# serval/kaboodle

Hardware: AMD Instinct MI355X
Metric: simulated peer-rounds/sec (whole node) + rounds to fingerprint convergence (higher is better)
Workload: dtype u8

## Files before the change

include/kaboodle_sim.h:

```cpp
#ifndef KABOODLE_SIM_H
#define KABOODLE_SIM_H

#include <stddef.h>
#include <stdint.h>

#ifdef __cplusplus
extern "C" {
#endif

#define KB_ABI_VERSION 3u

enum {
  KB_OK = 0,
  KB_INVALID_OPERATION = 1,
  KB_IO_ERROR = 2,
  KB_NO_DEVICE = 3,
  KB_STOPPING_FAILED = 4,
  KB_INVALID_ARGUMENT = 5,
  KB_CAPACITY = 6
};

enum { KB_INIT_JOIN = 0,
       KB_INIT_CONVERGED = 1 };

enum { KB_FAILED_SIM_SENDER = 0,
       KB_FAILED_SOCKET_FAITHFUL = 1 };

typedef struct kb_config {
  uint32_t abi_version;
  uint32_t capacity;
  uint32_t initial_nodes;
  uint32_t init_mode;
  uint64_t seed;
  uint32_t loss_threshold;
  uint32_t churn_threshold;
  int32_t  fault_end_round;
  uint32_t max_waves;
  uint32_t failed_mode;
  uint32_t id_len;
  uint32_t partition_groups;
  int32_t  partition_start;
  int32_t  partition_end;
  int32_t  device;
  uint32_t debug_flags;
  uint32_t track_latency;
  uint32_t variant;
  uint32_t sparse_row_cap;
  uint32_t stat_flags;
  uint32_t reserved[1];
} kb_config;
enum { KB_STAT_NO_SF_FAILED_DROPS = 1u };
enum { KB_VARIANT_SAME_WINDOW_BCAST = 1u,
       KB_VARIANT_EXACT_LRU = 2u,
       KB_VARIANT_SPARSE_ROWS = 4u };

enum {
  KB_DBG_PHASEB_HBM = 1u,
  KB_DBG_RESP_HBM = 2u,
  KB_DBG_KP_HBM = 4u,
  KB_DBG_KP_BIG_SMALL = 8u,
  KB_DBG_PROC_UNSORTED = 16u,
  KB_DBG_WAVE_GRAPH = 32u,
  KB_DBG_RESP_WAVE_HBM = 64u,
  KB_DBG_NO_UNION = 128u,
  KB_DBG_A3X_KPL8 = 256u,
  KB_DBG_A3X_WIDE = 512u,
  KB_DBG_WAVE0_SERIAL = 1024u
};

enum { KB_STATE_KNOWN = 0, KB_STATE_WAITING_FOR_PING = 1, KB_STATE_WAITING_FOR_INDIRECT_PING = 2 };
typedef struct kb_peer_state {
  uint32_t peer;
  uint32_t state;
  int32_t  since;
  uint32_t latency_ms;
  uint32_t identity_len;
  uint8_t  identity[32];
} kb_peer_state;
#define KB_LATENCY_NONE 0xFFFFFFFFu

typedef struct kb_stats {
  int32_t  round;
  uint32_t alive;
  uint32_t agree;
  int32_t  first_converged_round;
  int32_t  last_converged_round;
  uint32_t next_free_id;
  uint64_t sent_ping, sent_ping_req, sent_ack, sent_known_peers, sent_kpr;
  uint64_t bcast_join, bcast_failed;
  uint64_t drop_dead, drop_loss, drop_window, drop_oversize, drop_partition, drop_bcast;
  uint64_t removed_timeout, removed_failed, join_responses, curious_overflow, churn_leaves, churn_joins;
  uint64_t sent_kp_ids;
  uint64_t alive_rounds;
  uint64_t probe_responses;
  uint64_t exported;
  uint64_t reserved[4];
} kb_stats;

typedef struct kb_sim kb_sim;

void kb_config_default(kb_config* cfg);

int  kb_sim_create(const kb_config* cfg, kb_sim** out);
int  kb_sim_destroy(kb_sim* sim);
int  kb_sim_step(kb_sim* sim, uint32_t rounds);

int  kb_sim_start_node(kb_sim* sim, uint32_t node);
int  kb_sim_stop_node(kb_sim* sim, uint32_t node);
int  kb_sim_restart_node(kb_sim* sim, uint32_t node, uint32_t* new_node);
int  kb_sim_is_running(kb_sim* sim, uint32_t node, int* running);
int  kb_sim_ping_addrs(kb_sim* sim, uint32_t node, const uint32_t* peers, size_t n);
int  kb_sim_set_identity(kb_sim* sim, uint32_t node, const uint8_t* identity, size_t len);
int  kb_sim_identity(kb_sim* sim, uint32_t node, uint8_t* buf, size_t cap, size_t* len);

int  kb_sim_fingerprint(kb_sim* sim, uint32_t node, uint32_t* fp);
int  kb_sim_fingerprints(kb_sim* sim, uint32_t* fps, size_t cap);
int  kb_sim_peers(kb_sim* sim, uint32_t node, uint32_t* peers, size_t cap, size_t* n);
int  kb_sim_peer_states(kb_sim* sim, uint32_t node, kb_peer_state* out, size_t cap, size_t* n);
int  kb_sim_stats(kb_sim* sim, kb_stats* out);
int  kb_sim_true_fingerprint(kb_sim* sim, uint32_t* fp);

int  kb_sim_watch(kb_sim* sim, uint32_t node);
int  kb_sim_events(kb_sim* sim, uint32_t node, uint32_t* discovered, size_t cap_d, size_t* n_d,
                   uint32_t* departed, size_t cap_p, size_t* n_p, uint32_t* fp, int* fp_changed);

typedef struct kb_wire_addr { uint8_t ip[4]; uint16_t port; uint16_t pad; } kb_wire_addr;

typedef struct kb_probe_response {
  uint32_t responder;
  uint32_t probe;
  int32_t  round;
  kb_wire_addr prober;
  uint32_t identity_len;
  uint8_t  identity[32];
} kb_probe_response;
int  kb_sim_probe(kb_sim* sim, const kb_wire_addr* prober);
int  kb_sim_probe_responses(kb_sim* sim, kb_probe_response* out, size_t cap, size_t* n);
typedef struct kb_broadcast { uint32_t kind, sender, peer, pad; } kb_broadcast;
int  kb_sim_broadcasts(kb_sim* sim, kb_broadcast* out, size_t cap, size_t* n);

typedef struct kb_unicast {
  int32_t  round;
  uint32_t wave, sender, dest, seq, kind, a, fp, n, pay_off, pay_len, pad;
} kb_unicast;
int  kb_sim_set_external(kb_sim* sim, uint32_t node);
int  kb_sim_inject(kb_sim* sim, const kb_unicast* msg, const uint32_t* ids);
int  kb_sim_exported(kb_sim* sim, kb_unicast* out, size_t cap, size_t* n, uint32_t* ids, size_t cap_ids, size_t* n_ids);

#define KB_UNIQUE_ID_BYTES 128
int  kb_rccl_unique_id(uint8_t* out, size_t cap);
int  kb_ipc_unique_id(uint8_t* out, size_t cap);
int  kb_sim_create_rank(const kb_config* cfg, int32_t rank, int32_t world, const uint8_t* unique_id,
                        kb_sim** out);
int  kb_sim_create_local(const kb_config* cfg, int32_t shards, kb_sim** out);
int  kb_sim_shard_info(kb_sim* sim, int32_t* rank, int32_t* world, uint32_t* lo, uint32_t* hi);

int  kb_sim_dump_row(kb_sim* sim, uint32_t node, uint8_t* row, size_t cap);
int  kb_sim_dump_scalars(kb_sim* sim, int32_t* out, size_t cap);
int  kb_sim_dump_suspects(kb_sim* sim, uint32_t node, int32_t* out, size_t cap, size_t* n);
int  kb_sim_debug_paths(kb_sim* sim, uint32_t* mask);
int  kb_sim_debug_counters(kb_sim* sim, uint64_t* out, size_t cap);
int  kb_sim_dump_curious(kb_sim* sim, uint32_t node, int32_t* out, size_t cap, size_t* n);
int  kb_sim_sparse_footprint(kb_sim* sim, uint64_t* out, size_t cap);
int  kb_sim_dump_checkpoints(kb_sim* sim, uint32_t node, uint32_t seg[128], uint64_t* stale, uint32_t* dirty,
                             uint32_t* fp_cached);
enum { KB_FOLD_TICK = 0, KB_FOLD_FP_ALL = 1, KB_FOLD_FP_ONE = 2, KB_FOLD_THREAD = 3 };
typedef struct kb_fold_probe {
  uint32_t path, split, nrows, pad;
  const uint32_t* rows;
  const uint8_t*  running;
  const uint32_t* bits;
  const uint64_t* stale;
  const uint32_t* segp_in;
  uint32_t* segp_out;
  uint64_t* stale_out;
  uint32_t* dirty_out;
  uint32_t* fp_out;
  uint64_t* fold_bytes;
} kb_fold_probe;
int  kb_sim_debug_fold(kb_sim* sim, const kb_fold_probe* p);

int  kb_format_addr(uint32_t id, char* buf, size_t cap);
uint32_t kb_fingerprint_of_set(const uint32_t* ids, size_t n, const uint8_t* identities,
                               size_t id_stride, const uint8_t* id_lens);

const char* kb_last_error(void);

enum { KB_WIRE_PING = 0, KB_WIRE_PING_REQUEST = 1, KB_WIRE_ACK = 2, KB_WIRE_KNOWN_PEERS = 3,
       KB_WIRE_KNOWN_PEERS_REQUEST = 4,
       KB_WIRE_JOIN = 16, KB_WIRE_FAILED = 17, KB_WIRE_PROBE = 18,
       KB_WIRE_PROBE_RESPONSE = 32 };
enum { KB_WIRE_CHANNEL_UNICAST = 0, KB_WIRE_CHANNEL_BROADCAST = 1, KB_WIRE_CHANNEL_PROBE_RESPONSE = 2 };
typedef struct kb_wire_entry { kb_wire_addr addr; uint32_t id_off, id_len; } kb_wire_entry;
typedef struct kb_wire_msg {
  uint32_t kind;
  uint32_t identity_off, identity_len;
  kb_wire_addr peer;
  uint32_t fingerprint, num_peers;
  uint32_t n_entries;
} kb_wire_msg;
int kb_wire_encode(const kb_wire_msg* m, const kb_wire_entry* entries, const uint8_t* idents, uint8_t* buf,
                   size_t cap, size_t* size);
int kb_wire_decode(const uint8_t* buf, size_t len, int channel, kb_wire_msg* m, kb_wire_entry* entries, size_t cap);
int kb_wire_addr_of_id(uint32_t id, kb_wire_addr* out);
int kb_wire_id_of_addr(const kb_wire_addr* addr, uint32_t* id);

enum { KB_KT_ROWPASS = 0,
       KB_KT_ROUND = 1,
       KB_KT_FOLD = 2,
       KB_KT_RESP = 3,
       KB_KT_PROC = 4 };
int  kb_sim_kernel_time(kb_sim* sim, int kind, double* ms, uint64_t* launches);
int  kb_sim_reset_kernel_time(kb_sim* sim);
int  kb_sim_kernel_bytes(kb_sim* sim, int kind, uint64_t* bytes);
#define KB_WAVE_SLOTS 9
typedef struct kb_kernel_time {
  char     name[24];
  double   ms;
  uint64_t launches;
  uint64_t bytes;
// ... 12 lines not shown
```

kaboodle_amd/_ffi.py:

```python
from __future__ import annotations

import ctypes as C
import os
from dataclasses import dataclass

KB_ABI_VERSION = 3
KB_OK, KB_INVALID_OPERATION, KB_IO_ERROR, KB_NO_DEVICE, KB_STOPPING_FAILED, KB_INVALID_ARGUMENT, KB_CAPACITY = range(7)
KB_INIT_JOIN, KB_INIT_CONVERGED = 0, 1
KB_FAILED_SIM_SENDER, KB_FAILED_SOCKET_FAITHFUL = 0, 1
KB_DBG_PHASEB_HBM, KB_DBG_RESP_HBM, KB_DBG_KP_HBM, KB_DBG_KP_BIG_SMALL, KB_DBG_PROC_UNSORTED = 1, 2, 4, 8, 16
KB_DBG_ALL = 31
KB_DBG_WAVE_GRAPH = 32
KB_DBG_RESP_WAVE_HBM = 64
KB_DBG_NO_UNION = 128
KB_DBG_A3X_KPL8 = 256
KB_DBG_A3X_WIDE = 512
KB_DBG_WAVE0_SERIAL = 1024
KB_VARIANT_SAME_WINDOW_BCAST, KB_VARIANT_EXACT_LRU = 1, 2
KB_STAT_NO_SF_FAILED_DROPS = 1
KB_VARIANT_SPARSE_ROWS = 4
KB_LATENCY_NONE = 0xFFFFFFFF
KT_ROWPASS, KT_ROUND, KT_FOLD, KT_RESP, KT_PROC = 0, 1, 2, 3, 4
KB_WAVE_SLOTS = 9
STATE_NAMES = {0: "Known", 1: "WaitingForPing", 2: "WaitingForIndirectPing"}


class KbConfig(C.Structure):
    _fields_ = [
        ("abi_version", C.c_uint32), ("capacity", C.c_uint32), ("initial_nodes", C.c_uint32),
        ("init_mode", C.c_uint32), ("seed", C.c_uint64), ("loss_threshold", C.c_uint32),
        ("churn_threshold", C.c_uint32), ("fault_end_round", C.c_int32), ("max_waves", C.c_uint32),
        ("failed_mode", C.c_uint32), ("id_len", C.c_uint32), ("partition_groups", C.c_uint32),
        ("partition_start", C.c_int32), ("partition_end", C.c_int32), ("device", C.c_int32),
        ("debug_flags", C.c_uint32), ("track_latency", C.c_uint32), ("variant", C.c_uint32),
        ("sparse_row_cap", C.c_uint32), ("stat_flags", C.c_uint32), ("reserved", C.c_uint32 * 1),
    ]


class KbPeerState(C.Structure):
    _fields_ = [("peer", C.c_uint32), ("state", C.c_uint32), ("since", C.c_int32), ("latency_ms", C.c_uint32),
                ("identity_len", C.c_uint32), ("identity", C.c_uint8 * 32)]


PEER_STATE_DTYPE = [("peer", "<u4"), ("state", "<u4"), ("since", "<i4"), ("latency_ms", "<u4"), ("identity_len", "<u4"),
                    ("identity", "u1", (32,))]


class KbStats(C.Structure):
    _fields_ = [
        ("round", C.c_int32), ("alive", C.c_uint32), ("agree", C.c_uint32),
        ("first_converged_round", C.c_int32), ("last_converged_round", C.c_int32), ("next_free_id", C.c_uint32),
        ("sent_ping", C.c_uint64), ("sent_ping_req", C.c_uint64), ("sent_ack", C.c_uint64),
        ("sent_known_peers", C.c_uint64), ("sent_kpr", C.c_uint64),
        ("bcast_join", C.c_uint64), ("bcast_failed", C.c_uint64),
        ("drop_dead", C.c_uint64), ("drop_loss", C.c_uint64), ("drop_window", C.c_uint64),
        ("drop_oversize", C.c_uint64), ("drop_partition", C.c_uint64), ("drop_bcast", C.c_uint64),
        ("removed_timeout", C.c_uint64), ("removed_failed", C.c_uint64), ("join_responses", C.c_uint64),
        ("curious_overflow", C.c_uint64), ("churn_leaves", C.c_uint64), ("churn_joins", C.c_uint64),
        ("sent_kp_ids", C.c_uint64), ("alive_rounds", C.c_uint64), ("probe_responses", C.c_uint64),
        ("exported", C.c_uint64), ("reserved", C.c_uint64 * 4),
    ]

    def as_dict(self) -> dict:
        return {n: getattr(self, n) for n, _ in self._fields_ if n != "reserved"}


class KbKernelTime(C.Structure):
    _fields_ = [("name", C.c_char * 24), ("ms", C.c_double), ("launches", C.c_uint64), ("bytes", C.c_uint64),
                ("has_bytes", C.c_uint32), ("pad", C.c_uint32), ("wave_ms", C.c_double * KB_WAVE_SLOTS)]


KB_CENSUS_NONE = 0xFFFFFFFF


def _summary(st: C.Structure, lists=()) -> dict:
    return {n: [int(x) for x in getattr(st, n)] if n in lists else int(getattr(st, n))
            for n, _ in st._fields_ if n not in ("reserved", "pad")}


def diff_results(a, b, array_names) -> list[str]:
    import numpy as np
    out = [f"summary.{k}: {v} != {b.summary[k]}" for k, v in a.summary.items() if b.summary[k] != v]
    for name in array_names:
        x, y = getattr(a, name), getattr(b, name)
        if (x is None) != (y is None):
            out.append(f"{name}: only one side has the array")
        elif x is not None and not np.array_equal(x, y):
            if x.ndim > 1 or x.shape != y.shape:
                out.append(f"{name}: {len(x)} listed != {len(y)} listed, or other entries")
            else:
                bad = np.flatnonzero(x != y)
                out.append(f"{name}: {len(bad)} differ, first id {bad[0]}: {x[bad[0]]} != {y[bad[0]]}")
    return out


_PTR = {"u4": C.POINTER(C.c_uint32), "i4": C.POINTER(C.c_int32), "u8": C.POINTER(C.c_uint64)}


def _out_arrays(arrays: bool, *groups):
    import numpy as np
    outs, args = [], []
    for dtypes, n in groups:
        made = [np.zeros(n, dtype=dt) if arrays else None for dt in dtypes]
        outs += made
        args += [m.ctypes.data_as(_PTR[dt]) if arrays else None for m, dt in zip(made, dtypes)]
        args.append(n if arrays else 0)
    return outs, args


class KbCensus(C.Structure):
    _fields_ = [("round", C.c_int32), ("observers", C.c_uint32), ("running", C.c_uint32), ("exact_views", C.c_uint32),
                ("pairs", C.c_uint64), ("missing", C.c_uint64), ("stale", C.c_uint64),
                ("full_ids", C.c_uint32), ("ghost_ids", C.c_uint32), ("least_known", C.c_uint32),
                ("least_known_by", C.c_uint32), ("top_ghost", C.c_uint32), ("top_ghost_by", C.c_uint32),
                ("reserved", C.c_uint64 * 4)]

    def as_dict(self) -> dict:
        return _summary(self)


class KbReciprocity(C.Structure):
    _fields_ = [("round", C.c_int32), ("observers", C.c_uint32), ("mutual_pairs", C.c_uint64),
                ("oneway_pairs", C.c_uint64), ("rows_mutual", C.c_uint32), ("rows_oneway", C.c_uint32),
                ("max_mutual_row", C.c_uint32), ("max_mutual", C.c_uint32), ("pairs_listed", C.c_uint64),
                ("reserved", C.c_uint64 * 4)]

    def as_dict(self) -> dict:
        return _summary(self)


class KbFpClass(C.Structure):
    _fields_ = [("fp", C.c_uint32), ("size", C.c_uint32), ("rep", C.c_uint32), ("pad", C.c_uint32)]


class KbFpClasses(C.Structure):
    _fields_ = [("round", C.c_int32), ("observers", C.c_uint32), ("classes", C.c_uint32), ("largest", C.c_uint32),
                ("singletons", C.c_uint32), ("true_fp", C.c_uint32), ("true_size", C.c_uint32),
                ("true_rank", C.c_uint32), ("size_hist", C.c_uint32 * 32), ("listed", C.c_uint32),
                ("listed_observers", C.c_uint32), ("reserved", C.c_uint64 * 4)]

    def as_dict(self) -> dict:
        d = _summary(self, ("size_hist",))
        d["size_hist"] = d.pop("size_hist")
        return d


KB_FPC_LIST_MAX = 1024
_FPC_OUT = [C.POINTER(KbFpClasses), C.POINTER(KbFpClass), C.c_size_t, C.POINTER(C.c_size_t), C.POINTER(C.c_uint32),
            C.POINTER(C.c_uint32), C.c_size_t]


class KbLatCensus(C.Structure):
    _fields_ = [("round", C.c_int32), ("observers", C.c_uint32), ("measured", C.c_uint64), ("sum_ms", C.c_uint64),
                ("min_ms", C.c_uint32), ("max_ms", C.c_uint32), ("max_peer", C.c_uint32), ("measured_ids", C.c_uint32),
                ("hist", C.c_uint64 * 17), ("orphans", C.c_uint64), ("reserved", C.c_uint64 * 4)]

    def as_dict(self) -> dict:
        return _summary(self, ("hist",))


_LATC_OUT = [C.POINTER(KbLatCensus), C.POINTER(C.c_uint32), C.POINTER(C.c_uint64), C.POINTER(C.c_uint32),
             C.POINTER(C.c_uint32), C.c_size_t, C.POINTER(C.c_uint32), C.POINTER(C.c_uint64), C.c_size_t]


class KbAgeCensus(C.Structure):
    _fields_ = [("round", C.c_int32), ("observers", C.c_uint32), ("cells", C.c_uint64), ("suspects", C.c_uint64),
                ("ancient", C.c_uint64), ("windowed", C.c_uint64), ("fresh", C.c_uint64), ("dead_suspects", C.c_uint64),
                ("dead_ancient", C.c_uint64), ("dead_windowed", C.c_uint64), ("dead_fresh", C.c_uint64),
                ("unheard_ids", C.c_uint32), ("oldest_heard_id", C.c_uint32), ("oldest_heard", C.c_int32),
                ("pad", C.c_uint32), ("hist", C.c_uint64 * 256), ("reserved", C.c_uint64 * 4)]
# ... 773 lines not shown
```

kaboodle_amd/csrc/kb_common.h:

```cpp
#pragma once
#include "kb_device.h"
#include "../../include/kaboodle_sim.h"

namespace kb {

enum StatIdx {
  S_PING, S_PINGREQ, S_ACK, S_KP, S_KPR, S_BJOIN, S_BFAIL, S_DEAD, S_LOSS, S_WINDOW, S_OVERSIZE, S_PART, S_BDROP,
  S_RMTIMEOUT, S_RMFAILED, S_JRESP, S_CUROVF, S_CLEAVE, S_CJOIN,
  S_KPIDS,
  S_ROWB,
  S_FOLDB,
  S_A3ROWS, S_A3DEEP, S_A3CHUNKS,
  S_ALIVER,
  S_RESPB,
  S_PROCB,
  S_PROBERESP,
  S_EXPORT,
  S_A3X32, S_A3XCLAMP, S_A3XFEW, S_A3XLIVE, S_A3XWIDE,
  NSTAT
};
enum CtrIdx {
  C_KP, C_SLOW, C_ACTIVE, C_AGREE, C_ALIVE, C_LEAVES, C_NEXTFREE, C_ERR, C_FIRSTCONV, C_LASTCONV, C_LASTAGREE,
  C_LASTALIVE, C_DBG_INS, C_DBG_FP, C_DBG_MAXFP,
  C_DBG_KPR, C_DBG_KPRLOG, C_DBG_BASE,
  C_DBG_TNODE, C_DBG_TMAX, C_DBG_TBASE, C_DBG_TINS,
  C_DBG_TSTART, C_DBG_TEND, C_DBG_MSGS,
  C_TICK,
  C_ROUND,
  C_PATHS,
  C_DBG_SLOW_LONG, C_DBG_SLOW_NONMEM, C_DBG_SLOW_DIRTY, C_DBG_SLOW_KPR, C_DBG_SLOW_OTHER,
  C_RESTN,
  C_XREC, C_XPAY,
  NCTR
};
enum : uint32_t { PATH_PHASEB_HBM = 1, PATH_RESP_SCRATCH_SAMPLED = 2, PATH_RESP_SCRATCH_FULL = 4, PATH_KP_BIG_HBM = 8,
                  PATH_PROC_UNSORTED = 16, PATH_BFAIL_PREP_HBM = 32, PATH_RESP_WAVE = 64, PATH_KP_BIG_LDS = 128,
                  PATH_RESP_WAVE_HBM = 256,
                  PATH_PROC_DEFERRED = 512,
                  PATH_ROWPASS_LDS_HBM_LISTS = 1024,
                  PATH_KPR_WRAPPED = 2048,
                  PATH_RESP_JOINERS_HBM = 4096,
                  PATH_JOIN_LIST_PAST_UCAP = 8192 };
constexpr int NSEG = 64;
constexpr int ZT = 9;
constexpr int ZB = 9 * 1024;

struct Dev {
  uint32_t lo, hi;
  uint32_t C, W, SEGW, NWR;
  uint32_t segq, segm;
  uint32_t k0, k1;
  uint32_t loss_thr, churn_thr;
  int32_t fault_end;
  uint32_t failed_mode;
  uint32_t pgroups;
  int32_t pstart, pend;
  uint32_t uniform, L;
  uint32_t capk, capj;
  uint32_t paybound;
  uint32_t dbg;
  uint32_t dev;
  uint8_t* stamp;
  uint32_t* bits;
  uint2* segp;
  unsigned long long* sdirty;
  uint8_t* dirty;
  uint8_t* alive;
  uint8_t* idset;
  uint32_t* abits;
  int32_t* start_round;
  uint32_t* n;
  uint32_t* fp;
  int32_t* last_bcast;
  uint32_t* a3cur;
  Susp* susp;
  Cur* cur;
  uint32_t* paq;
  uint32_t* paq_n;
  uint32_t* cseg;
  uint32_t* segmul;
  uint32_t* seglen;
  uint32_t* zpow;
  uint32_t* zfin;
  uint32_t* ztab;
  uint32_t* zbtab;
  uint32_t* htab;
  unsigned long long* stats;
  unsigned long long* sacc;
  uint32_t* ctr;
  uint32_t* truefp;
  uint2* tfpart;
  uint32_t* flog;
  uint32_t* flog_n;
  uint32_t* fstart;
  int32_t* kpr_big;
  uint16_t* lat;
  int32_t wave;
  uint8_t* ext;
  struct XRec* xrec;
  uint32_t* xids;
  uint32_t xrec_cap, xids_cap;
  int32_t* tst;
  int32_t* tlb;
};

struct XRec { int32_t round; uint32_t wave, sender, dest, seq, kind, a, fp, n, pay_off, pay_len, pad; };
constexpr uint32_t DERR_EXPORT = 11;
__device__ inline void export_rec(uint32_t* ctr, XRec* xrec, uint32_t xrec_cap, uint32_t* xids, uint32_t xids_cap,
                                  const Msg& m, const uint32_t* pay, int32_t r, uint32_t w) {
  const uint32_t k = atomicAdd(&ctr[C_XREC], 1u);
  const uint32_t np = m.kind == K_KP ? m.a : 0u;
  const uint32_t po = np ? atomicAdd(&ctr[C_XPAY], np) : 0u;
  if (k >= xrec_cap || po + np > xids_cap) { atomicCAS(&ctr[C_ERR], 0u, DERR_EXPORT); return; }
  for (uint32_t q = 0; q < np; ++q) xids[po + q] = pay[m.off + q];
  xrec[k] = XRec{r, w, m.sender, m.dest, m.seq, m.kind, m.kind == K_KP ? 0u : m.a, m.fp, m.n, po, np, 0u};
}

__device__ inline uint32_t log_entry(uint32_t peer, int32_t r) { return (peer << 8) | ((uint32_t)r & 255u); }
__device__ inline int32_t log_round(uint32_t e, int32_t r) { return r - (int32_t)(((uint32_t)r - (e & 255u)) & 255u); }
__device__ inline uint32_t log_window_start(const Dev& d, uint32_t i, int32_t r) {
  return r >= SHARE_AGE - 1 ? d.fstart[(size_t)i * 16 + ((uint32_t)(r - (SHARE_AGE - 1)) & 15u)] : 0u;
}
typedef __attribute__((address_space(3))) void lds_void_t;
typedef __attribute__((address_space(1))) void glb_void_t;
__device__ __attribute__((always_inline)) inline void stage16(uint4* dst, const uint4* src, uint32_t n, uint32_t t,
                                                             uint32_t lanes) {
  const uint32_t wb = t - lane();
  for (uint32_t w0 = 0; wb + w0 < n; w0 += lanes) {
    if (t + w0 < n)
      __builtin_amdgcn_global_load_lds((glb_void_t*)(src + t + w0), (lds_void_t*)(dst + wb + w0), 16, 0, 0);
  }
  __builtin_amdgcn_s_waitcnt(0x0F70);
  asm volatile("" ::: "memory");
}
__device__ __attribute__((always_inline)) inline void copy16(uint4* dst, const uint4* src, uint32_t n, uint32_t t,
                                                            uint32_t lanes) {
  constexpr int U = 8;
  uint32_t w0 = t;
  for (; w0 + lanes * (U - 1) < n; w0 += lanes * U) {
    uint4 v[U];
#pragma unroll
    for (int u = 0; u < U; ++u) v[u] = src[w0 + lanes * u];
#pragma unroll
    for (int u = 0; u < U; ++u) dst[w0 + lanes * u] = v[u];
  }
  for (; w0 < n; w0 += lanes) dst[w0] = src[w0];
}
constexpr uint32_t PIN_WORDS = 1024;
constexpr uint32_t PIN_SEQ = PIN_WORDS - 1;
__device__ inline void pin_publish(uint32_t* h, const uint32_t* v, uint32_t n, uint32_t seq) {
  for (uint32_t k = 0; k < n; ++k) h[k] = v[k];
  if (!seq) return;
  __threadfence_system();
  __hip_atomic_store(h + PIN_SEQ, seq, __ATOMIC_RELEASE, __HIP_MEMORY_SCOPE_SYSTEM);
}
__device__ inline int32_t round_of(const Dev& d, int32_t r_arg) {
  return r_arg >= 0 ? r_arg : (int32_t)__builtin_amdgcn_readfirstlane(d.ctr[C_ROUND]);
}
__device__ inline void set_err(const Dev& d, uint32_t e) { atomicCAS(&d.ctr[C_ERR], 0u, e); }
__device__ inline void path_hit(const Dev& d, uint32_t bit) {
  if (!(__hip_atomic_load(&d.ctr[C_PATHS], __ATOMIC_RELAXED, __HIP_MEMORY_SCOPE_AGENT) & bit)) atomicOr(&d.ctr[C_PATHS], bit);
}
__device__ inline bool faults(const Dev& d, int32_t r) { return d.fault_end < 0 || r < d.fault_end; }
__device__ inline bool local(const Dev& d, uint32_t i) { return i >= d.lo && i < d.hi; }
__device__ inline bool part_blocks(const Dev& d, int32_t r, uint32_t a, uint32_t b) {
  if (d.pgroups <= 1 || r < d.pstart || r >= d.pend) return false;
  return ((uint64_t)a * d.pgroups / d.C) != ((uint64_t)b * d.pgroups / d.C);
}
__device__ inline uint8_t* row_of(const Dev& d, uint32_t i) { return d.stamp + (size_t)i * d.W; }
__device__ inline uint32_t* bits_of(const Dev& d, uint32_t i) { return d.bits + (size_t)i * d.NWR; }
__device__ inline bool is_mem(const Dev& d, uint32_t i, uint32_t j) { return (bits_of(d, i)[j >> 5] >> (j & 31)) & 1u; }
__device__ inline uint32_t seg_of(const Dev& d, uint32_t j) { return d.segq == 1 ? (j >> 7) : __umulhi(j >> 7, d.segm); }
__device__ inline unsigned long long seg_bit(const Dev& d, uint32_t j) { return 1ull << seg_of(d, j); }
__device__ inline bool mem_set(const Dev& d, uint32_t i, uint32_t j) {
  const uint32_t m = 1u << (j & 31);
  return !(atomicOr(&bits_of(d, i)[j >> 5], m) & m);
}
__device__ inline bool mem_clr(const Dev& d, uint32_t i, uint32_t j) {
  const uint32_t m = 1u << (j & 31);
  return (atomicAnd(&bits_of(d, i)[j >> 5], ~m) & m) != 0;
}
__device__ inline void mark(const Dev& d, uint32_t i, unsigned long long segs) {
  if (segs) { atomicOr(&d.sdirty[i], segs); d.dirty[i] = 1; }
}

__device__ inline uint32_t mulzc(const uint32_t* tab, uint32_t x, uint32_t c) {
  if (c == 0) return x;
  const uint32_t* t = tab + c * 128;
  return t[x & 15] ^ t[16 + ((x >> 4) & 15)] ^ t[32 + ((x >> 8) & 15)] ^ t[48 + ((x >> 12) & 15)] ^
         t[64 + ((x >> 16) & 15)] ^ t[80 + ((x >> 20) & 15)] ^ t[96 + ((x >> 24) & 15)] ^ t[112 + (x >> 28)];
}
__device__ inline uint32_t mulzb(const uint32_t* tab, uint32_t x, uint32_t c) {
  const uint32_t* t = tab + c * 1024;
  return t[x & 255] ^ t[256 + ((x >> 8) & 255)] ^ t[512 + ((x >> 16) & 255)] ^ t[768 + (x >> 24)];
}
// ... 267 lines not shown
```

kaboodle_amd/csrc/kb_round.h:

```cpp
#pragma once
#include "kb_common.h"

namespace kb {

__global__ void k_rebase(Dev d, int32_t r) {
  const size_t total = (size_t)(d.hi - d.lo) * d.W / 16;
  const uint32_t wpr = d.W / 16;
  const int32_t E = epoch_base(r - 1);
  uint4* p = reinterpret_cast<uint4*>(d.stamp + (size_t)d.lo * d.W);
  for (size_t k = (size_t)blockIdx.x * blockDim.x + threadIdx.x; k < total; k += (size_t)gridDim.x * blockDim.x) {
    const uint4 v = p[k];
    uint32_t w[4] = {v.x, v.y, v.z, v.w};
    bool any = false;
#pragma unroll
    for (int q = 0; q < 4; ++q) {
      uint32_t x = w[q], y = 0;
#pragma unroll
      for (int t = 0; t < 4; ++t) {
        uint32_t b = (x >> (8 * t)) & 0xFF;
        if (b > ST_ANCIENT) {
          if (d.tst && b <= ST_ANCIENT + EPOCH) {
            const size_t i = d.lo + k / wpr, j = (k % wpr) * 16 + q * 4 + t;
            d.tst[i * d.W + j] = (int32_t)b - EOFF + E;
            atomicMin(d.tlb + i * (d.W >> 10) + (j >> 10), (int32_t)b - EOFF + E);
// ... 952 lines not shown
#pragma unroll
  for (int j = 0; j < 6; ++j) v[j] = SP[l2 + j < h2 ? l2 + j : h2];
  if (v[0] <= b && b < v[5]) {
    uint32_t c = 0, bs = v[0];
#pragma unroll
    for (int j = 1; j < 5; ++j) { const bool le = v[j] <= b; c += le; bs = le ? v[j] : bs; }
    *base = bs;
    return l2 + c;
  }
  uint32_t lo = 0, hi = nblk;
  while (hi - lo > 1) { const uint32_t mid = (lo + hi) >> 1; if (SP[mid] <= b) lo = mid; else hi = mid; }
  *base = SP[lo];
  return lo;
}
__device__ __attribute__((always_inline)) inline uint32_t block_pick(const uint4& q0, const uint4& q1, uint32_t blk,
                                                                     uint32_t rem) {
  const uint32_t p0 = __popc(q0.x), p1 = __popc(q0.y), p2 = __popc(q0.z), p3 = __popc(q0.w);
  const uint32_t p4 = __popc(q1.x), p5 = __popc(q1.y), p6 = __popc(q1.z);
  const uint32_t s01 = p0 + p1, s45 = p4 + p5, s03 = s01 + p2 + p3;
  const bool h1 = rem >= s03;
  rem -= h1 ? s03 : 0u;
  const uint32_t sa = h1 ? s45 : s01;
  const bool h2 = rem >= sa;
  rem -= h2 ? sa : 0u;
  const uint32_t pa = h1 ? (h2 ? p6 : p4) : (h2 ? p2 : p0);
  const bool h3 = rem >= pa;
  rem -= h3 ? pa : 0u;
  const uint32_t wi = (h1 ? 4u : 0u) + (h2 ? 2u : 0u) + (h3 ? 1u : 0u);
  const uint32_t xa = h1 ? (h2 ? (h3 ? q1.w : q1.z) : (h3 ? q1.y : q1.x)) : (h2 ? (h3 ? q0.w : q0.z) : (h3 ? q0.y : q0.x));
  return (blk * 8 + wi) * 32 + select_in_word(xa, rem);
}
__device__ inline uint32_t bm_select(const uint32_t* S, const uint32_t* SP, uint32_t nblk, float ratio, uint32_t b) {
  uint32_t base;
  const uint32_t lo = bm_block(SP, nblk, ratio, b, &base);
  const uint4 q0 = *reinterpret_cast<const uint4*>(S + lo * 8), q1 = *reinterpret_cast<const uint4*>(S + lo * 8 + 4);
  return block_pick(q0, q1, lo, b - base);
}
constexpr uint32_t KB_RESP_U = 2;
constexpr int RESP_U = KB_RESP_U;
constexpr int RESP_KMAX = 9;
struct JoinLds {
  const uint32_t *J, *JM;
  __device__ uint32_t min_from(uint32_t u) const { return JM[u]; }
  __device__ uint32_t at(uint32_t f) const { return J[f]; }
};
struct JoinRegs {
  uint32_t j0, j1, jmin;
  __device__ uint32_t min_from(uint32_t) const { return jmin; }
  __device__ uint32_t at(uint32_t f) const { return f < 64 ? rdl(j0, (int)f) : rdl(j1, (int)(f - 64)); }
};
template <class JA>
__device__ __attribute__((always_inline)) inline void sampled_fill(uint32_t* pay, uint32_t k_first, uint32_t stride,
                                                                   uint32_t cap, const Prp& P, const uint32_t* B,
                                                                   const uint32_t* BP, uint32_t NB, float ratio,
                                                                   const JA& J, uint32_t upto, uint32_t nnew) {
  const uint32_t jmin = J.min_from(upto);
  const uint32_t mcount = k_first < cap ? (cap - k_first + stride - 1) / stride : 0u;
  uint32_t y[RESP_KMAX];
#pragma unroll
  for (int q = 0; q < RESP_KMAX; ++q) y[q] = 0;
  if (4ull * P.n >= 3ull * ((uint64_t)(P.ma + 1) << P.c)) {
#pragma unroll
    for (int q = 0; q < RESP_KMAX; ++q) {
      const bool act = (uint32_t)q < mcount;
      if (!__ballot(act)) break;
      uint32_t x = prp_pass(k_first + stride * q, P);
      while (__ballot(act && x >= P.n)) { if (act && x >= P.n) x = prp_pass(x, P); }
      y[q] = x;
    }
  } else {
    uint32_t m = 0, x = k_first;
    while (__ballot(m < mcount)) {
      if (m < mcount) {
        x = prp_pass(x, P);
        if (x < P.n) {
#pragma unroll
          for (int q = 0; q < RESP_KMAX; ++q) if ((uint32_t)q == m) y[q] = x;
          ++m;
          x = k_first + stride * m;
        }
      }
    }
  }
#pragma unroll
  for (int q0 = 0; q0 < RESP_KMAX; q0 += RESP_U) {
    if ((uint32_t)q0 >= mcount) break;
    uint32_t blk[RESP_U], bb[RESP_U];
    uint4 b0[RESP_U], b1[RESP_U];
#pragma unroll
    for (int u = 0; u < RESP_U; ++u) {
      bb[u] = 0;
      blk[u] = q0 + u < RESP_KMAX ? bm_block(BP, NB, ratio, y[q0 + u < RESP_KMAX ? q0 + u : 0], &bb[u]) : 0u;
    }
#pragma unroll
    for (int u = 0; u < RESP_U; ++u) {
      b0[u] = *reinterpret_cast<const uint4*>(B + blk[u] * 8);
      b1[u] = *reinterpret_cast<const uint4*>(B + blk[u] * 8 + 4);
    }
#pragma unroll
    for (int u = 0; u < RESP_U; ++u) {
      const uint32_t q = q0 + u;
      if (q >= RESP_KMAX || q >= mcount) break;
      const uint32_t yq = y[q];
      uint32_t xq = block_pick(b0[u], b1[u], blk[u], yq - bb[u]);
      if (xq >= jmin) {
        uint32_t e = 0;
        while (true) {
          uint32_t c = 0;
          for (uint32_t f = upto; f < nnew; ++f) c += J.at(f) <= xq;
          if (c == e) break;
          e = c;
          xq = bm_select(B, BP, NB, ratio, yq + e);
        }
      }
      pay[k_first + stride * q] = xq;
    }
  }
}
constexpr uint32_t RESP_LDS_W = 131072;
constexpr uint32_t RESP_JCAP = 1024;
__host__ __device__ inline size_t resp_words(uint32_t NW, uint32_t NB) {
  return (2ull * NW + 2ull * (NB + 1) + 2ull * RESP_JCAP + 1 + 3) & ~3ull;
}

__device__ __attribute__((always_inline)) inline uint32_t block_prefix(const uint32_t* X, uint32_t* XP, uint32_t NB, uint32_t* s_red) {
  const uint32_t t = threadIdx.x, T = blockDim.x;
  const uint32_t per = (NB + T - 1) / T;
  uint32_t bc = 0;
  for (uint32_t k = t * per; k < (t + 1) * per && k < NB; ++k) {
    uint32_t c = 0;
    for (uint32_t w = 0; w < 8; ++w) c += __popc(X[k * 8 + w]);
    XP[k] = c; bc += c;
  }
  uint32_t ex = wave_excl(bc);
  const uint32_t wt = wave_sum(bc);
  __syncthreads();
  if (lane() == 0) s_red[t >> 6] = wt;
  __syncthreads();
  for (uint32_t w = 0; w < (t >> 6); ++w) ex += s_red[w];
  uint32_t tot = 0;
  for (uint32_t w = 0; w < T / 64; ++w) tot += s_red[w];
  for (uint32_t k = t * per; k < (t + 1) * per && k < NB; ++k) { const uint32_t c = XP[k]; XP[k] = ex; ex += c; }
  if (t == 0) XP[NB] = tot;
  __syncthreads();
  return tot;
}

constexpr uint32_t RW_JCAP = 128;
__host__ __device__ inline uint32_t rwave_head(uint32_t NB) { return ((NB + 1 > RW_JCAP ? NB + 1 : RW_JCAP) + 3) & ~3u; }
__host__ __device__ inline uint32_t rwave_words(uint32_t NW, uint32_t NB) { return rwave_head(NB) + NW; }
__device__ inline bool resp_by_wave(const Dev& d, uint32_t i, uint32_t nnew, bool on) {
  return on && d.uniform && nnew <= RW_JCAP && d.n[i] - nnew > d.capj;
}
template <bool SG>
__global__ __launch_bounds__(256) __attribute__((amdgpu_waves_per_eu(4))) void k_resp_wave(Dev d, PhaseB pb, const uint32_t* nodes, const uint32_t* nnodes_p,
                                                   OutBuf ob, int32_t r, uint32_t* rest) {
  extern __shared__ __attribute__((aligned(16))) uint32_t rw_lds[];
  const uint32_t NW = d.NWR, NB = d.W / 256;
  const uint32_t wv = threadIdx.x >> 6, l = lane(), nwv = blockDim.x >> 6;
  uint32_t* BP = rw_lds + (size_t)wv * (SG ? rwave_head(NB) : rwave_words(NW, NB));
  uint32_t* Jt = BP;
  uint32_t* S = BP + rwave_head(NB);
  const uint32_t nnodes = *nnodes_p;
  const bool small_lists = pb.JW <= 64 && pb.nj <= 128;
  const uint32_t js0 = small_lists && l < pb.nj ? pb.bjoin[l].sender : 0u;
  const uint32_t js1 = small_lists && l + 64 < pb.nj ? pb.bjoin[l + 64].sender : 0u;
  const uint32_t stride = gridDim.x * nwv;
  uint32_t it = blockIdx.x * nwv + wv;
  uint32_t inext = it < nnodes ? nodes[it] : 0u;
  for (; it < nnodes; it += stride) {
    const uint32_t i = inext;
    const unsigned long long* nm = pb.newmask + (size_t)i * pb.JW;
    const unsigned long long* rm = pb.respmask + (size_t)i * pb.JW;
    const unsigned long long nmv = small_lists && l < pb.JW ? nm[l] : 0ull;
    const unsigned long long rmv = small_lists && l < pb.JW ? rm[l] : 0ull;
    const uint32_t n_i = d.n[i], nbase_i = pb.nbase[i], poff_i = ob.poff[i], ooff_i = ob.off[i];
    inext = it + stride < nnodes ? nodes[it + stride] : 0u;
    const uint32_t* B = bits_of(d, i);
    const uint4* B4 = reinterpret_cast<const uint4*>(B);
    const bool tdbg = (d.dev & 512) != 0;
    const uint64_t tps = tdbg ? wall_clock64() : 0;
    if (!SG) stage16(reinterpret_cast<uint4*>(S), B4, NW / 4, l, 64);
    uint32_t nnew = 0;
    if (small_lists) nnew = wave_sum((uint32_t)__popcll(nmv));
    else for (uint32_t wj = 0; wj < pb.JW; ++wj) nnew += __popcll(nm[wj]);
    if (!(d.uniform && nnew <= RW_JCAP && n_i - nnew > d.capj)) {
      if (l == 0) rest[atomicAdd(&d.ctr[C_RESTN], 1u)] = i;
      wait_lds();
      __builtin_amdgcn_wave_barrier();
      continue;
    }
    if (l == 0) path_hit(d, SG ? PATH_RESP_WAVE_HBM : PATH_RESP_WAVE);
    uint64_t tp0 = tdbg ? wall_clock64() : 0, tp1 = 0, tp2 = 0;
    if (small_lists) {
      const unsigned long long w0 = ((unsigned long long)rdl((uint32_t)(nmv >> 32), 0) << 32) | rdl((uint32_t)nmv, 0);
      const unsigned long long w1 = ((unsigned long long)rdl((uint32_t)(nmv >> 32), 1) << 32) | rdl((uint32_t)nmv, 1);
      if (l < pb.nj && ((w0 >> l) & 1ull)) Jt[__popcll(w0 & ((1ull << l) - 1ull))] = js0;
      if (l + 64 < pb.nj && ((w1 >> l) & 1ull)) Jt[__popcll(w0) + __popcll(w1 & ((1ull << l) - 1ull))] = js1;
    } else {
      for (uint32_t e = l; e < pb.nj; e += 64) {
        if (!newbit(nm, e)) continue;
        uint32_t pos = __popcll(nm[e >> 6] & ((1ull << (e & 63)) - 1ull));
        for (uint32_t w2 = 0; w2 < (e >> 6); ++w2) pos += __popcll(nm[w2]);
        Jt[pos] = pb.bjoin[e].sender;
      }
    }
    wait_lds();
    __builtin_amdgcn_wave_barrier();
    const uint32_t jr0 = l < nnew ? Jt[l] : 0xFFFFFFFFu, jr1 = l + 64 < nnew ? Jt[l + 64] : 0xFFFFFFFFu;
    uint32_t sm0 = jr0, sm1 = jr1;
#pragma unroll
    for (int o = 1; o < 64; o <<= 1) {
      const uint32_t u0 = __shfl_down(sm0, o, 64), u1 = __shfl_down(sm1, o, 64);
      if (l + o < 64) { sm0 = u0 < sm0 ? u0 : sm0; sm1 = u1 < sm1 ? u1 : sm1; }
    }
    {
      const uint32_t m1 = rdl(sm1, 0);
      sm0 = m1 < sm0 ? m1 : sm0;
    }
    wait_lds();
    __builtin_amdgcn_wave_barrier();
    if (tdbg) tp1 = wall_clock64();
    const uint32_t per = (NB + 63) / 64;
    uint32_t bc = 0, last = 0;
    const uint4* S4 = reinterpret_cast<const uint4*>(SG ? B : S);
    for (uint32_t k = l * per; k < (l + 1) * per && k < NB; ++k) {
      const uint4 q0 = S4[2 * k], q1 = S4[2 * k + 1];
      const uint32_t c = __popc(q0.x) + __popc(q0.y) + __popc(q0.z) + __popc(q0.w) + __popc(q1.x) + __popc(q1.y) +
                         __popc(q1.z) + __popc(q1.w);
      BP[k] = c; bc += c;
      if (c) last = k + 1;
    }
    uint32_t ex = wave_excl(bc);
    const uint32_t nB = wave_sum(bc);
    const uint32_t nbu = wave_max(last);
    const float ratio = nB ? (float)nbu / (float)nB : 0.0f;
    for (uint32_t k = l * per; k < (l + 1) * per && k < NB; ++k) { const uint32_t c = BP[k]; BP[k] = ex; ex += c; }
    if (l == 0) BP[NB] = nB;
    wait_lds();
    __builtin_amdgcn_wave_barrier();
    uint32_t poff = poff_i, q = 0, ins_before = 0;
    if (tdbg) tp2 = wall_clock64();
    for (uint32_t wj = 0; wj < pb.JW; ++wj) {
      unsigned long long rmw, nmw;
      if (small_lists) {
        rmw = ((unsigned long long)rdl((uint32_t)(rmv >> 32), (int)wj) << 32) | rdl((uint32_t)rmv, (int)wj);
        nmw = ((unsigned long long)rdl((uint32_t)(nmv >> 32), (int)wj) << 32) | rdl((uint32_t)nmv, (int)wj);
      } else {
        rmw = rm[wj]; nmw = nm[wj];
      }
      while (rmw) {
        const uint32_t bit = (uint32_t)(__ffsll((long long)rmw) - 1);
        const uint32_t K = wj * 64 + bit;
        rmw &= rmw - 1;
        const uint32_t upto = ins_before + __popcll(nmw & ((2ull << bit) - 1ull));
        const uint32_t expect = nbase_i + upto;
        const uint32_t a = small_lists ? (K < 64 ? rdl(js0, (int)K) : rdl(js1, (int)(K - 64))) : pb.bjoin[K].sender;
        const uint32_t nk = nB - (nnew - upto), cap = d.capj;
        uint32_t* pay = ob.pay + poff;
        const Prp P = prp_make(nk, philox(i, (uint32_t)r, (uint32_t)P_TRUNC << 24, a, d.k0, d.k1));
        const uint32_t jmin = upto < 64 ? rdl(sm0, (int)upto) : upto < 128 ? rdl(sm1, (int)(upto - 64)) : 0xFFFFFFFFu;
        sampled_fill(pay, l, 64, cap, P, SG ? B : S, BP, NB, ratio, JoinRegs{jr0, jr1, jmin}, upto, nnew);
        if (l == 0) {
          Msg m; m.dest = a; m.sender = i; m.seq = q; m.kind = K_KP; m.a = cap; m.fp = 0; m.n = 0; m.off = poff;
          ob.msgs[ooff_i + q] = m;
          if (nk != expect) set_err(d, DERR_RESP);
        }
        poff += cap; q++;
      }
      ins_before += __popcll(nmw);
    }
    if (l == 0) slot_add(d, S_RESPB, 4ull * NW + 16ull * pb.JW + 4ull * pb.nj + (4ull * d.capj + 32ull) * q +
                                     (SG ? 32ull * d.capj * q : 0ull));
    if (tdbg && l == 0) {
      __builtin_amdgcn_s_waitcnt(0);
      const uint64_t tp3 = wall_clock64();
      atomicAdd(&d.ctr[C_DBG_TNODE], (uint32_t)(tp2 - tp1)); atomicAdd(&d.ctr[C_DBG_TBASE], (uint32_t)(tp1 - tp0));
      atomicAdd(&d.ctr[C_DBG_TINS], (uint32_t)(tp3 - tp2)); atomicAdd(&d.ctr[C_DBG_TSTART], 1u);
      atomicAdd(&d.ctr[C_DBG_MSGS], q); atomicAdd(&d.ctr[C_DBG_TEND], (uint32_t)(tp0 - tps));
    }
    wait_lds();
    __builtin_amdgcn_wave_barrier();
  }
}

__global__ __launch_bounds__(256) void k_resp_node(Dev d, PhaseB pb, const uint32_t* nodes, const uint32_t* nnodes_p,
                                                   OutBuf ob, int32_t r, uint32_t* gscratch, bool wave_on) {
  extern __shared__ uint32_t lds_dyn[];
  const uint32_t NW = d.NWR, NB = d.W / 256;
  uint32_t* lds = gscratch ? gscratch + (size_t)blockIdx.x * resp_words(NW, NB) : lds_dyn;
  uint32_t* B = lds;
  uint32_t* BP = B + NW;
  uint32_t* S = BP + NB + 1;
  uint32_t* SP = S + NW;
  uint32_t* J = SP + NB + 1;
  uint32_t* JM = J + RESP_JCAP;
  __shared__ uint32_t s_red[16];
  const uint32_t t = threadIdx.x, T = blockDim.x;
  const uint32_t nnodes = *nnodes_p;
  for (uint32_t it = blockIdx.x; it < nnodes; it += gridDim.x) {
    const uint32_t i = nodes[it];
    const unsigned long long* nm = pb.newmask + (size_t)i * pb.JW;
    const unsigned long long* rm = pb.respmask + (size_t)i * pb.JW;
    uint32_t nnew = 0;
    for (uint32_t wj = 0; wj < pb.JW; ++wj) nnew += __popcll(nm[wj]);
    if (resp_by_wave(d, i, nnew, wave_on)) continue;
    if (gscratch) copy16(reinterpret_cast<uint4*>(B), reinterpret_cast<const uint4*>(bits_of(d, i)), NW / 4, t, T);
    else stage16(reinterpret_cast<uint4*>(B), reinterpret_cast<const uint4*>(bits_of(d, i)), NW / 4, t, T);
    __syncthreads();
    const uint32_t nB = block_prefix(B, BP, NB, s_red);
    const bool jl = nnew <= RESP_JCAP;
    if (jl) {
      for (uint32_t e = t; e < pb.nj; e += T) {
        if (!newbit(nm, e)) continue;
        uint32_t pos = __popcll(nm[e >> 6] & ((1ull << (e & 63)) - 1ull));
        for (uint32_t w2 = 0; w2 < (e >> 6); ++w2) pos += __popcll(nm[w2]);
        J[pos] = pb.bjoin[e].sender;
      }
      __syncthreads();
      if (nnew <= T) {
        uint32_t v = t < nnew ? J[t] : 0xFFFFFFFFu;
#pragma unroll
        for (int o = 1; o < 64; o <<= 1) {
          const uint32_t u = __shfl_down(v, o, 64);
          if (lane() + o < 64) v = u < v ? u : v;
        }
        if (lane() == 0) s_red[t >> 6] = v;
        __syncthreads();
        for (uint32_t w = (t >> 6) + 1; w < T / 64; ++w) v = s_red[w] < v ? s_red[w] : v;
        if (t < nnew) JM[t] = v;
        if (t == 0) JM[nnew] = 0xFFFFFFFFu;
      } else if (t == 0) {
        uint32_t m = 0xFFFFFFFFu;
        JM[nnew] = m;
        for (uint32_t q3 = nnew; q3 > 0; --q3) { m = J[q3 - 1] < m ? J[q3 - 1] : m; JM[q3 - 1] = m; }
      }
    }
    __syncthreads();
    uint32_t poff = ob.poff[i], q = 0, ins_before = 0;
    for (uint32_t wj = 0; wj < pb.JW; ++wj) {
      unsigned long long rmw = rm[wj];
      const unsigned long long nmw = nm[wj];
      while (rmw) {
        const uint32_t bit = (uint32_t)(__ffsll((long long)rmw) - 1);
        const uint32_t K = wj * 64 + bit;
        rmw &= rmw - 1;
        const uint32_t upto = ins_before + __popcll(nmw & ((2ull << bit) - 1ull));
        const uint32_t expect = pb.nbase[i] + upto;
        const uint32_t a = pb.bjoin[K].sender;
        const uint32_t nk = nB - (nnew - upto);
        const bool sample = d.uniform && nk > d.capj;
        const uint32_t cap = sample ? d.capj : nk;
        uint32_t* pay = ob.pay + poff;
        if (sample) {
          const Prp P = prp_make(nk, philox(i, (uint32_t)r, (uint32_t)P_TRUNC << 24, a, d.k0, d.k1));
          const float ratio = nB ? (float)NB / (float)nB : 0.0f;
          if (jl) {
            sampled_fill(pay, t, T, cap, P, B, BP, NB, ratio, JoinLds{J, JM}, upto, nnew);
          } else {
            for (uint32_t k = t; k < cap; k += T) {
              const uint32_t y = prp_eval(k, P);
              uint32_t e = 0, x;
              while (true) {
                x = bm_select(B, BP, NB, ratio, y + e);
                uint32_t c = 0;
                for (uint32_t f = K + 1; f < pb.nj; ++f)
                  if (newbit(nm, f)) c += pb.bjoin[f].sender <= x;
                if (c == e) break;
                e = c;
              }
              pay[k] = x;
            }
          }
        } else {
          for (uint32_t k = t; k < NW; k += T) S[k] = B[k];
          __syncthreads();
          for (uint32_t f = K + 1 + t; f < pb.nj; f += T)
            if (newbit(nm, f)) { const uint32_t x = pb.bjoin[f].sender; atomicAnd(&S[x >> 5], ~(1u << (x & 31))); }
          __syncthreads();
          block_prefix(S, SP, NB, s_red);
          for (uint32_t w = t; w < NW; w += T) {
            uint32_t x = S[w];
            if (!x) continue;
            uint32_t pos = bm_rank(S, SP, w * 32);
            while (x) { const uint32_t b = __ffs(x) - 1; x &= x - 1; pay[pos++] = w * 32 + b; }
          }
        }
        if (t == 0) {
          Msg m; m.dest = a; m.sender = i; m.seq = q; m.kind = K_KP; m.a = cap; m.fp = 0; m.n = 0; m.off = poff;
          ob.msgs[ob.off[i] + q] = m;
          if (nk != expect) set_err(d, DERR_RESP);
          if (gscratch) path_hit(d, sample ? PATH_RESP_SCRATCH_SAMPLED : PATH_RESP_SCRATCH_FULL);
          if (!jl) path_hit(d, PATH_RESP_JOINERS_HBM);
        }
        poff += cap; q++;
        __syncthreads();
      }
      ins_before += __popcll(nmw);
    }
  }
}

}
```

kaboodle_amd/csrc/kb_sim.hip:

```cpp
#include <hip/hip_runtime.h>
#include <hip/hip_ext.h>
#include <stdint.h>
#include <stdio.h>
#include <string.h>
#include <stdlib.h>
#include <string>
#include <vector>
#include <array>
#include <algorithm>
#include <atomic>
#include <thread>
#include "kb_common.h"
#include "kb_wire.h"
#include "kb_round.h"
#include "kb_tick.h"
#include "kb_waves.h"
#include "kb_xfer.h"
#include "kb_sparse.h"

using namespace kb;

enum KId : int {
  KI_REBASE, KI_EVENTS, KI_CHURN_LEAVE, KI_CHURN_JOIN, KI_ALIVE_BITS, KI_TRUEFP_PART, KI_TRUEFP_FIN, KI_LOG_MARK,
  KI_LAT_MARK, KI_BFAIL_PREP, KI_ROWPASS, KI_LAT_SWEEP, KI_SCAN_TILES, KI_SCAN_APPLY, KI_SET_CAP, KI_RESP_WAVE,
  KI_RESP_NODE, KI_TICK_SCAN, KI_TICK_PRE, KI_FOLD, KI_FP_ROWS, KI_TICK_POST, KI_BCAST_WRITE, KI_ROUTE, KI_ROUTE_X,
  KI_XBOUND, KI_PACK, KI_ROUTE_RECV, KI_SCATTER, KI_SCATTER_FLAT, KI_KP, KI_SORTFAST, KI_PROC, KI_ROUND_END,
  KI_PROBE, KI_A3_EXACT, NKI
};
static const char* const KNAME[NKI] = {
  "k_rebase", "k_events", "k_churn_leave", "k_churn_join", "k_alive_bits", "k_truefp_part", "k_truefp_fin",
  "k_log_mark", "k_lat_mark", "k_bfail_prep", "k_rowpass", "k_lat_sweep", "k_scan_tiles", "k_scan_apply",
  "k_set_cap", "k_resp_wave", "k_resp_node", "k_tick_scan", "k_tick_pre", "k_fold", "k_fp_rows", "k_tick_post",
  "k_bcast_write", "k_route", "k_route_x", "k_xbound", "k_pack", "k_route_recv", "k_scatter", "k_scatter_flat",
  "k_kp", "k_sortfast", "k_proc", "k_round_end", "k_probe", "k_a3_exact"};
static int kbytes_stat(int kid) {
  switch (kid) {
    case KI_ROWPASS: return S_ROWB;
    case KI_FOLD: return S_FOLDB;
    case KI_RESP_WAVE: return S_RESPB;
    case KI_PROC: return S_PROCB;
    default: return -1;
  }
}

struct ScanArgs {
  const uint32_t* in[4]; uint32_t* out[4]; int narr; uint32_t n;
  uint32_t* totals;
  uint32_t* list; uint32_t* list_count; uint32_t list_base;
  uint32_t list_or3;
  uint32_t addc[4];
  uint32_t* tiles;
  uint32_t ntiles;
};
__device__ inline uint32_t scan_val(const ScanArgs& a, int q, uint32_t j) {
  if (q == 4) return a.in[0][j] != 0 || (a.list_or3 && a.in[3][j] != 0);
  return (a.in[q] ? a.in[q][j] : 0) + a.addc[q];
}
__global__ __launch_bounds__(1024) void k_scan_tiles(ScanArgs a) {
  __shared__ uint32_t red[5][16];
  const uint32_t j = blockIdx.x * 1024 + threadIdx.x;
  const int nq = a.list ? 5 : a.narr;
  for (int q = 0; q < 5; ++q) {
    if (q >= a.narr && !(q == 4 && a.list)) continue;
    uint32_t v = j < a.n ? scan_val(a, q, j) : 0;
    v = wave_sum(v);
    if (lane() == 0) red[q][threadIdx.x >> 6] = v;
  }
  __syncthreads();
  if (threadIdx.x < 5 && (threadIdx.x < (uint32_t)a.narr || (threadIdx.x == 4 && a.list))) {
    uint32_t t = 0;
    for (int w = 0; w < 16; ++w) t += red[threadIdx.x][w];
    a.tiles[threadIdx.x * a.ntiles + blockIdx.x] = t;
  }
  (void)nq;
}
__global__ __launch_bounds__(1024) void k_scan_apply(ScanArgs a) {
  __shared__ uint32_t base[5], red[5][16], wpre[5][16];
  const uint32_t tile = blockIdx.x, t = threadIdx.x;
  const uint32_t j = tile * 1024 + t;
  for (int q = 0; q < 5; ++q) {
    const bool on = q < a.narr || (q == 4 && a.list);
    uint32_t s = 0;
    if (on) for (uint32_t k = t; k < tile; k += 1024) s += a.tiles[q * a.ntiles + k];
    s = wave_sum(s);
    if (lane() == 0) red[q][t >> 6] = s;
  }
  __syncthreads();
  if (t < 5) { uint32_t s = 0; for (int w = 0; w < 16; ++w) s += red[t][w]; base[t] = s; }
  __syncthreads();
  uint32_t v[5], ex[5];
  for (int q = 0; q < 5; ++q) {
    const bool on = q < a.narr || (q == 4 && a.list);
    v[q] = (on && j < a.n) ? scan_val(a, q, j) : 0;
    ex[q] = wave_excl(v[q]);
    const uint32_t tot = wave_sum(v[q]);
    if (lane() == 0) wpre[q][t >> 6] = tot;
  }
  __syncthreads();
  if (t < 5) { uint32_t run = 0; for (int w = 0; w < 16; ++w) { uint32_t x = wpre[t][w]; wpre[t][w] = run; run += x; } }
  __syncthreads();
  for (int q = 0; q < a.narr; ++q) if (j < a.n) a.out[q][j] = base[q] + wpre[q][t >> 6] + ex[q];
  if (a.list && j < a.n && v[4]) a.list[base[4] + wpre[4][t >> 6] + ex[4]] = j + a.list_base;
  if (tile == gridDim.x - 1 && t == 1023) {
    for (int q = 0; q < a.narr; ++q) a.totals[q] = base[q] + wpre[q][15] + ex[q] + v[q];
    if (a.list) { const uint32_t c = base[4] + wpre[4][15] + ex[4] + v[4]; a.totals[4] = c; if (a.list_count) *a.list_count = c; }
  }
}


__global__ void k_build_htab(Dev d) {
  const size_t k = (size_t)blockIdx.x * blockDim.x + threadIdx.x;
  const size_t total = (size_t)(d.W / 8) * 256;
  if (k >= total) return;
  const uint32_t h = (uint32_t)(k >> 8), m = (uint32_t)(k & 255);
  uint32_t raw = 0;
  for (uint32_t t = 0; t < 8; ++t) {
    const uint32_t j = h * 8 + t;
    if (((m >> t) & 1u) && j < d.C) raw = multmodp(d.zpow[1], raw) ^ d.cseg[j];
  }
  d.htab[k] = raw;
}
__global__ void k_set_cap(Dev d, const uint32_t* nresp, uint32_t* cap, uint32_t* cnt, const uint32_t* tot, uint32_t* hpin,
                          uint32_t seq) {
  const uint32_t i = d.lo + blockIdx.x * blockDim.x + threadIdx.x;
  if (i < d.hi) { cap[i] = nresp[i] + TICK_MAX; cnt[i] = nresp[i]; }
  if (blockIdx.x == 0 && threadIdx.x == 0) { d.ctr[C_RESTN] = 0; pin_publish(hpin, tot, 5, seq); }
}
__global__ void k_publish(const uint32_t* v, uint32_t n, uint32_t* hpin, uint32_t seq) {
  if (blockIdx.x == 0 && threadIdx.x == 0) pin_publish(hpin, v, n, seq);
}
__global__ void k_init_nodes(Dev d, uint32_t n0) {
  const uint32_t i = blockIdx.x * blockDim.x + threadIdx.x;
  if (i >= d.C) return;
  if (local(d, i)) { d.last_bcast[i] = NONE_ROUND; d.a3cur[i] = i; }
  d.start_round[i] = NONE_ROUND;
  if (i < n0) node_start(d, i, 0);
}
__global__ void k_init_converged_rows(Dev d, uint32_t n0) {
  const uint32_t wpr = d.W / 16;
  const uint32_t r0 = d.lo, r1 = n0 < d.hi ? n0 : d.hi;
  const size_t words = r1 > r0 ? (size_t)(r1 - r0) * wpr : 0;
  uint4* p = reinterpret_cast<uint4*>(d.stamp);
  for (size_t k = (size_t)blockIdx.x * blockDim.x + threadIdx.x; k < words; k += (size_t)gridDim.x * blockDim.x) {
    const uint32_t i = r0 + (uint32_t)(k / wpr), c = (uint32_t)(k % wpr);
    uint32_t w4[4];
    for (int q = 0; q < 4; ++q) {
      uint32_t y = 0;
      for (int t = 0; t < 4; ++t) {
        const uint32_t j = c * 16 + q * 4 + t;
        uint32_t b = j < n0 ? ST_ANCIENT : 0;
        if (j == i) b = enc(0, 0);
        y |= b << (8 * t);
      }
      w4[q] = y;
    }
    p[(size_t)i * wpr + c] = make_uint4(w4[0], w4[1], w4[2], w4[3]);
  }
  const size_t bw = r1 > r0 ? (size_t)(r1 - r0) * d.NWR : 0;
  for (size_t k = (size_t)blockIdx.x * blockDim.x + threadIdx.x; k < bw; k += (size_t)gridDim.x * blockDim.x) {
    const uint32_t w = (uint32_t)(k % d.NWR);
    uint32_t x = 0;
    if (w * 32 + 32 <= n0) x = 0xFFFFFFFFu;
    else if (w * 32 < n0) x = (1u << (n0 - w * 32)) - 1u;
    d.bits[(size_t)r0 * d.NWR + k] = x;
  }
}
__global__ void k_init_converged_nodes(Dev d, uint32_t n0) {
  const uint32_t i = blockIdx.x * blockDim.x + threadIdx.x;
  if (i >= d.C) return;
  const bool loc = local(d, i);
  if (loc) { d.last_bcast[i] = NONE_ROUND; d.a3cur[i] = i; }
  d.start_round[i] = NONE_ROUND;
  if (i >= n0) return;
  d.alive[i] = 1; d.start_round[i] = 0;
  if (loc) { d.dirty[i] = 1; d.n[i] = n0; d.last_bcast[i] = -1000; d.paq_n[i] = 0; d.sdirty[i] = ~0ull; }
}
__global__ void k_mark_all_dirty(Dev d) {
  const uint32_t i = d.lo + blockIdx.x * blockDim.x + threadIdx.x;
  if (i < d.hi) { d.dirty[i] = 1; d.sdirty[i] = ~0ull; }
}
__global__ __launch_bounds__(64) void k_fp_one(Dev d, uint32_t i) {
  __shared__ uint32_t ztab[ZT * 128];
  load_ztab(d, ztab);
  if (!d.dirty[i]) return;
  const uint32_t f = wave_fp(d, ztab, i, 0);
  if (lane() == 0) { d.fp[i] = f; d.dirty[i] = 0; }
}
__global__ __launch_bounds__(256) void k_fp_all(Dev d) {
  __shared__ uint32_t ztab[ZT * 128];
  load_ztab(d, ztab);
  const uint32_t i = d.lo + blockIdx.x * 4 + (threadIdx.x >> 6);
  if (i >= d.hi || !d.dirty[i]) return;
  const uint32_t f = wave_fp(d, ztab, i, 0);
  if (lane() == 0) { d.fp[i] = f; d.dirty[i] = 0; }
}

static thread_local std::string g_err;
static void seterr(const std::string& s) { g_err = s; }
#define HIPCHK(x) do { hipError_t e_ = (x); if (e_ != hipSuccess) { seterr(std::string(#x) + ": " + hipGetErrorString(e_)); return KB_IO_ERROR; } } while (0)

template <class T> static hipError_t dalloc(T** p, size_t n) {
  hipError_t e = hipMalloc((void**)p, sizeof(T) * (n ? n : 1));
  if (e == hipSuccess) e = hipMemset(*p, 0, sizeof(T) * (n ? n : 1));
  if (e == hipSuccess) e = hipDeviceSynchronize();
  return e;
}

static int merge_ext_joins(hipStream_t st, BCast* list, uint32_t* n, std::vector<uint32_t>& joins, uint32_t pgroups, uint32_t C) {
  if (joins.empty()) return KB_OK;
  std::vector<BCast> v(*n);
  if (*n) HIPCHK(hipMemcpyAsync(v.data(), list, sizeof(BCast) * *n, hipMemcpyDeviceToHost, st));
  HIPCHK(hipStreamSynchronize(st));
  for (const uint32_t x : joins) {
    const uint32_t g = pgroups > 1 ? (uint32_t)((uint64_t)x * pgroups / C) : 0u;
    const auto at = std::upper_bound(v.begin(), v.end(), x, [](uint32_t a, const BCast& b) { return a < b.sender; });
    v.insert(at, BCast{x, x, 0, g});
  }
  HIPCHK(hipMemcpyAsync(list, v.data(), sizeof(BCast) * v.size(), hipMemcpyHostToDevice, st));
  HIPCHK(hipStreamSynchronize(st));
  *n = (uint32_t)v.size();
  joins.clear();
  return KB_OK;
}

static uint32_t h_crc_table[256];
static void h_crc_init() {
  for (uint32_t i = 0; i < 256; ++i) { uint32_t c = i; for (int k = 0; k < 8; ++k) c = (c & 1) ? (c >> 1) ^ CRC_POLY : c >> 1; h_crc_table[i] = c; }
}
static uint32_t h_crc_update(uint32_t reg, const uint8_t* p, size_t n) {
  for (size_t k = 0; k < n; ++k) reg = h_crc_table[(reg ^ p[k]) & 0xFF] ^ (reg >> 8);
  return reg;
}
static uint32_t h_xpow8(uint64_t n) {
  uint32_t res = 0x80000000u, sq = 0x00800000u;
  while (n) { if (n & 1) res = multmodp(sq, res); sq = multmodp(sq, sq); n >>= 1; }
  return res;
}

__global__ __launch_bounds__(1024) void k_events_diff(const uint32_t* __restrict__ row,
                                                      const uint32_t* __restrict__ snap, uint32_t C,
                                                      uint32_t* __restrict__ out) {
  __shared__ uint32_t wa[16], wr[16], base[2], known;
  const uint32_t t = threadIdx.x, lane = t & 63, wv = t >> 6, nw = (C + 31) / 32;
  uint32_t* add = out;
  uint32_t* rem = out + C;
  if (t == 0) { base[0] = 0; base[1] = 0; known = 0; }
  __syncthreads();
  uint32_t kn = 0;
  for (uint32_t w0 = 0; w0 < nw; w0 += 1024) {
    const uint32_t w = w0 + t;
    uint32_t cur = 0, old = 0;
    if (w < nw) {
      const uint32_t valid = (C - w * 32 >= 32) ? ~0u : ((1u << (C - w * 32)) - 1u);
      cur = row[w] & valid;
      old = snap[w] & valid;
    }
    const uint32_t a = cur & ~old, r = old & ~cur;
    kn += __popc(cur);
    uint32_t pa = __popc(a), pr = __popc(r);
    for (int o = 1; o < 64; o <<= 1) {
      const uint32_t xa = __shfl_up(pa, o, 64), xr = __shfl_up(pr, o, 64);
      if (lane >= (uint32_t)o) { pa += xa; pr += xr; }
    }
    if (lane == 63) { wa[wv] = pa; wr[wv] = pr; }
    __syncthreads();
    uint32_t oa = base[0] + pa - __popc(a), orr = base[1] + pr - __popc(r);
    for (uint32_t k = 0; k < wv; ++k) { oa += wa[k]; orr += wr[k]; }
    for (uint32_t m = a; m; m &= m - 1) add[oa++] = w * 32 + __ffs(m) - 1;
    for (uint32_t m = r; m; m &= m - 1) rem[orr++] = w * 32 + __ffs(m) - 1;
    __syncthreads();
    if (t == 1023) { base[0] = oa; base[1] = orr; }
    __syncthreads();
  }
  for (int o = 32; o > 0; o >>= 1) kn += __shfl_down(kn, o, 64);
  if (lane == 0) atomicAdd(&known, kn);
  __syncthreads();
  if (t == 0) { out[2 * C] = base[0]; out[2 * C + 1] = base[1]; out[2 * C + 2] = known; }
}
__global__ __launch_bounds__(256) void k_events_commit(const uint32_t* __restrict__ row, uint32_t* __restrict__ snap,
                                                       uint32_t nw) {
  const uint32_t w = blockIdx.x * 256 + threadIdx.x;
  if (w < nw) snap[w] = row[w];
}
__global__ __launch_bounds__(256) void k_lat_column(Dev d, uint32_t node, uint16_t* out) {
  const uint32_t j = blockIdx.x * 256 + threadIdx.x;
  if (j < d.C) out[j] = *lat_at(d, node, j);
}

namespace kb { struct SpSim; }
enum CensusMs { CM_VIEW, CM_RECIP, CM_CLASSES, CM_LAT, CM_AGE, CM_DELTA, CM_ISLANDS, CM_N };

struct kb_sim {
  kb_config cfg;
  SpSim* sp = nullptr;
  Dev d;
  int device;
  hipStream_t st;
  hipStream_t st2 = nullptr;
  hipEvent_t ev_fork[4] = {nullptr, nullptr, nullptr, nullptr}, ev_join[4] = {nullptr, nullptr, nullptr, nullptr};
  uint32_t C, W, S;
  uint32_t lo, hi, R;
  int rank, world;
  Xfer* xf;
  bool in_group;
  std::vector<void*> allocs;
  int32_t round;
  bool probed = false;
  std::vector<uint8_t> h_ident, h_idlen;
  std::vector<uint8_t> h_pend; std::vector<int16_t> h_pendlen;
  std::vector<uint8_t> h_moved;
  std::vector<uint8_t> h_idset;
  std::vector<uint8_t> h_ext;
  size_t n_ext = 0;
  std::vector<XRec> inj; std::vector<uint32_t> inj_ids;
  std::vector<uint32_t> inj_join;
  XRec* d_inj = nullptr; uint32_t* d_inj_ids = nullptr; size_t d_inj_cap = 0, d_inj_ids_cap = 0;
  std::vector<kb_unicast> xq; std::vector<uint32_t> xq_ids;
  std::vector<Event> events;
  uint32_t* rpack = nullptr; uint32_t* rpack_in = nullptr;
  std::vector<kb_wire_addr> probe_q, probes;
  std::vector<kb_probe_response> presp;
  uint2* d_presp = nullptr; uint32_t* d_presp_n = nullptr; size_t presp_cap = 0;
  OutBuf ob[2];
  WaveCtl wc;
  uint32_t msg_cap, pay_cap;
  BCast* bfail; BCast* bjoin;
  BCast* bfail_loc; BCast* bjoin_loc;
  uint32_t nf, nj;
  uint32_t ucap = 0;
  uint32_t host_paths = 0;
  uint64_t xbytes_cross = 0, xbytes_all = 0;
  BcastSlots bs;
  uint32_t* join_off; uint32_t* fail_off;
  uint32_t* scan_tot; uint32_t* scan_tiles;
  unsigned long long* newmask; unsigned long long* respmask; size_t mask_words;
  unsigned long long* newmask_base; unsigned long long* respmask_base;
  uint32_t* nresp; uint32_t* paysum; uint32_t* nbase; uint32_t* resp_off;
  uint32_t* resp_nodes; uint32_t* bf_gid; uint8_t* bf_dep;
  uint32_t* slow;
  uint32_t* defer = nullptr;
  uint32_t* w0ctr = nullptr;
  uint16_t* lat_col;
  uint32_t* fnamed;
  uint32_t* resp_scratch; size_t resp_scratch_words;
  RowOut ro;
  Event* d_events; size_t events_cap;
  XState xs;
  uint32_t* xall; unsigned long long* xstats;
  std::vector<uint32_t> h_xall;
  Msg* rmsg; uint32_t* rpay; uint8_t* rstatus; uint32_t* rinbox; uint32_t* rkp;
  size_t rmsg_cap, rpay_cap;
  double round_ms;
  uint32_t* rr = nullptr;
  uint64_t round_launches, bj_total, bf_total;
  struct KRec { int16_t kid, wave; hipEvent_t a, b; };
  int prof_level = 1;
  bool capturing = false;
  int cur_wave = -1;
  std::vector<hipEvent_t> ev_free;
  std::vector<KRec> krec;
  double k_ms[NKI] = {};
  double k_wms[NKI][KB_WAVE_SLOTS] = {};
  uint64_t k_n[NKI] = {};
  uint64_t k_bytes0[NSTAT] = {};
  uint64_t host_syncs = 0;
  uint32_t ncu = 256;
  uint32_t* cs_buf = nullptr;
  uint32_t* rc_buf = nullptr;
  uint2* rc_pairs = nullptr; size_t rc_pairs_cap = 0;
  char* fc_buf = nullptr; size_t fc_cap = 0;
  double census_ms[CM_N] = {};
  bool debug_waves = false;
  size_t lds_per_cu = 65536;
  std::vector<kb_sim*> shards;
  LocalHub* hub;
  std::vector<uint32_t> watch_node, watch_fp;
  std::vector<uint32_t*> watch_snap;
  uint32_t* ev_out = nullptr;
  uint32_t* h_pin = nullptr;
  uint32_t* d_pin = nullptr;
  uint32_t pin_seq = 0;
  uint64_t occ_key = ~0ull; int occ_val = 0;
  bool graph_on = false;
  hipGraph_t wave_graph = nullptr; hipGraphExec_t wave_exec = nullptr;
  uint64_t buf_gen = 0, wave_gen = ~0ull;
  uint32_t* lc_buf = nullptr;
  double sn_ms = 0;
  uint32_t* dl_base = nullptr;
  uint8_t* dl_run = nullptr;
  int32_t dl_round = 0;
  uint32_t* dl_buf = nullptr;
  uint32_t* is_buf = nullptr;
};

template <class T> static hipError_t talloc(kb_sim* s, T** p, size_t n) {
  hipError_t e = dalloc(p, n);
  if (e == hipSuccess) s->allocs.push_back((void*)*p);
  return e;
}
template <class T> static hipError_t eng_alloc(kb_sim* s, T** p, size_t n) { return talloc(s, p, n); }
static const char* eng_alloc_what(kb_sim*) { return "device allocation failed: "; }
template <class T> static T* bias(T* base, size_t per_row, uint32_t lo) {
  return reinterpret_cast<T*>(reinterpret_cast<uintptr_t>(base) - sizeof(T) * per_row * lo);
}
template <class T> static hipError_t ralloc(kb_sim* s, T** p, size_t per_row) {
  T* base = nullptr;
  hipError_t e = talloc(s, &base, per_row * s->R);
  *p = bias(base, per_row, s->lo);
  return e;
}
template <class T> static T* L(const kb_sim* s, T* p) { return p + s->lo; }

static void prof_events(kb_sim* s, int kid, hipEvent_t* a, hipEvent_t* b) {
  *a = *b = nullptr;
  if (s->capturing || s->prof_level <= 0 || (s->prof_level == 1 && (kbytes_stat(kid) < 0 || kid == KI_PROC))) return;
  hipEvent_t e[2];
  for (int k = 0; k < 2; ++k) {
    if (!s->ev_free.empty()) { e[k] = s->ev_free.back(); s->ev_free.pop_back(); }
    else if (hipEventCreate(&e[k]) != hipSuccess) { if (k) s->ev_free.push_back(e[0]); return; }
  }
  *a = e[0]; *b = e[1];
  const int w = s->cur_wave < 0 ? -1 : (s->cur_wave < KB_WAVE_SLOTS ? s->cur_wave : KB_WAVE_SLOTS - 1);
  s->krec.push_back(kb_sim::KRec{(int16_t)kid, (int16_t)w, e[0], e[1]});
}
template <typename F, typename... Args>
static void klaunch_on(kb_sim* s, hipStream_t stream, int kid, F kern, dim3 grid, dim3 block, uint32_t lds, Args... args) {
  hipEvent_t a, b;
  prof_events(s, kid, &a, &b);
  hipExtLaunchKernelGGL(kern, grid, block, lds, stream, a, b, 0, args...);
}
template <typename F, typename... Args>
static void klaunch(kb_sim* s, int kid, F kern, dim3 grid, dim3 block, uint32_t lds, Args... args) {
  klaunch_on(s, s->st, kid, kern, grid, block, lds, args...);
}
static void side_fork(kb_sim* s, int k) { (void)hipEventRecord(s->ev_fork[k], s->st); (void)hipStreamWaitEvent(s->st2, s->ev_fork[k], 0); }
static void side_done(kb_sim* s, int k) { (void)hipEventRecord(s->ev_join[k], s->st2); }
static void side_join(kb_sim* s, int k) { (void)hipStreamWaitEvent(s->st, s->ev_join[k], 0); }
static void prof_resolve(kb_sim* s, size_t n) {
  n = std::min(n, s->krec.size());
  for (size_t k = 0; k < n; ++k) {
    const kb_sim::KRec& q = s->krec[k];
    float ms = 0;
    hipError_t e = hipEventElapsedTime(&ms, q.a, q.b);
    if (e == hipErrorNotReady) {
      (void)hipGetLastError();
      (void)hipEventSynchronize(q.b);
      e = hipEventElapsedTime(&ms, q.a, q.b);
    }
    if (e == hipSuccess) {
      if (q.kid == NKI) { s->round_ms += ms; s->round_launches++; }
      else {
        s->k_ms[q.kid] += ms; s->k_n[q.kid]++;
        if (q.wave >= 0) s->k_wms[q.kid][q.wave] += ms;
      }
    }
    s->ev_free.push_back(q.a); s->ev_free.push_back(q.b);
  }
  s->krec.erase(s->krec.begin(), s->krec.begin() + n);
}

static ScanArgs scan_args(kb_sim* s, uint32_t n, uint32_t* totals) {
  ScanArgs a; memset(&a, 0, sizeof a); a.n = n; a.totals = totals;
  a.tiles = s->scan_tiles; a.ntiles = (n + 1023) / 1024; return a;
}
static void launch_scan(kb_sim* s, const ScanArgs& a) {
  if (!a.n) return;
  klaunch(s, KI_SCAN_TILES, k_scan_tiles, dim3(a.ntiles), dim3(1024), 0, a);
  klaunch(s, KI_SCAN_APPLY, k_scan_apply, dim3(a.ntiles), dim3(1024), 0, a);
}

extern "C" void kb_config_default(kb_config* c) {
  memset(c, 0, sizeof *c);
  c->abi_version = KB_ABI_VERSION; c->capacity = 1024; c->initial_nodes = 1024; c->init_mode = KB_INIT_JOIN;
  c->seed = 1; c->fault_end_round = -1; c->max_waves = 8; c->failed_mode = KB_FAILED_SIM_SENDER; c->device = -1;
}
extern "C" const char* kb_last_error(void) { return g_err.c_str(); }
extern "C" int kb_format_addr(uint32_t id, char* buf, size_t cap) {
  char tmp[32];
  int len = snprintf(tmp, sizeof tmp, "10.100.100.%u:%u", 100u + id / 50000u, 10000u + id % 50000u);
  if (!buf || cap < (size_t)len + 1) return KB_INVALID_ARGUMENT;
  memcpy(buf, tmp, (size_t)len + 1);
  return KB_OK;
}
static void default_identity(uint32_t id, uint32_t len, uint8_t* out) {
  for (uint32_t k = 0; k < len; ++k) out[k] = (uint8_t)('a' + ((id * 31u + k * 7u) % 26u));
}

static int upload_segments(kb_sim* s) {
  const uint32_t C = s->C;
  std::vector<uint32_t> cseg(C), segmul(C), seglen(C);
  bool uniform = true;
  uint32_t xp[ADDR_LEN + MAXID + 1];
  for (uint32_t l = 0; l <= ADDR_LEN + MAXID; ++l) xp[l] = h_xpow8(l);
  for (uint32_t j = 0; j < C; ++j) {
    char a[32]; kb_format_addr(j, a, sizeof a);
    uint32_t reg = h_crc_update(0, (const uint8_t*)a, ADDR_LEN);
    reg = h_crc_update(reg, &s->h_ident[(size_t)j * MAXID], s->h_idlen[j]);
    cseg[j] = reg; seglen[j] = ADDR_LEN + s->h_idlen[j]; segmul[j] = xp[seglen[j]];
    if (s->h_idlen[j] != s->cfg.id_len) uniform = false;
  }
  s->d.uniform = uniform ? 1 : 0;
  s->d.L = ADDR_LEN + s->cfg.id_len;
  const uint32_t Z = h_xpow8(s->d.L);
  std::vector<uint32_t> zpow(std::max<uint32_t>(C + 2, 17));
  zpow[0] = 0x80000000u;
  for (size_t k = 1; k < zpow.size(); ++k) zpow[k] = multmodp(Z, zpow[k - 1]);
  std::vector<uint32_t> ztab(17 * 128);
  for (uint32_t c = 0; c <= 16; ++c)
    for (uint32_t k = 0; k < 8; ++k)
      for (uint32_t v = 0; v < 16; ++v) ztab[c * 128 + k * 16 + v] = multmodp(zpow[c], v << (4 * k));
  HIPCHK(hipMemcpy(s->d.cseg, cseg.data(), 4ull * C, hipMemcpyHostToDevice));
  HIPCHK(hipMemcpy(s->d.segmul, segmul.data(), 4ull * C, hipMemcpyHostToDevice));
  HIPCHK(hipMemcpy(s->d.seglen, seglen.data(), 4ull * C, hipMemcpyHostToDevice));
  HIPCHK(hipMemcpy(s->d.zpow, zpow.data(), 4ull * (C + 2), hipMemcpyHostToDevice));
  {
    std::vector<uint32_t> zf(C + 2);
    for (uint32_t k = 0; k < C + 2; ++k) zf[k] = multmodp(zpow[k], 0xFFFFFFFFu);
    HIPCHK(hipMemcpy(s->d.zfin, zf.data(), 4ull * (C + 2), hipMemcpyHostToDevice));
  }
  HIPCHK(hipMemcpy(s->d.ztab, ztab.data(), 4ull * ztab.size(), hipMemcpyHostToDevice));
  std::vector<uint32_t> zb(ZB);
  for (uint32_t c = 0; c < 9; ++c)
    for (uint32_t k = 0; k < 4; ++k)
      for (uint32_t v = 0; v < 256; ++v) zb[c * 1024 + k * 256 + v] = multmodp(zpow[c], v << (8 * k));
  HIPCHK(hipMemcpy(s->d.zbtab, zb.data(), 4ull * zb.size(), hipMemcpyHostToDevice));
  const size_t hn = (size_t)(s->W / 8) * 256;
  k_build_htab<<<(unsigned)((hn + 255) / 256), 256>>>(s->d);
  HIPCHK(hipDeviceSynchronize());
  return KB_OK;
}

#include "kb_roundframe.h"
#include "kb_sparse_host.h"

static int sp_wrap(const kb_config* cfg, int rank, int world, Xfer* xf, kb_sim** out) {
  if (cfg->capacity == 0 || cfg->capacity > 7800000u || cfg->initial_nodes > cfg->capacity || cfg->id_len > MAXID ||
      cfg->max_waves == 0 || cfg->max_waves > 64) { seterr("config out of range"); delete xf; return KB_INVALID_ARGUMENT; }
  SpSim* sp = nullptr;
  const int rc = sp_create(cfg, rank, world, xf, &sp);
  if (rc) return rc;
  kb_sim* s = new kb_sim();
  s->cfg = *cfg; s->C = cfg->capacity; s->sp = sp; s->device = sp->device; s->rank = rank; s->world = world;
  s->lo = sp->lo; s->hi = sp->hi; s->R = sp->R;
  *out = s;
  return KB_OK;
}

static void free_all(kb_sim* s) {
  for (void* p : s->allocs) (void)hipFree(p);
  s->allocs.clear();
}
static void destroy_shard(kb_sim* s) {
  (void)hipSetDevice(s->device);
  if (s->st) (void)hipStreamSynchronize(s->st);
  free_all(s);
  for (auto& q : s->krec) { (void)hipEventDestroy(q.a); (void)hipEventDestroy(q.b); }
  for (hipEvent_t e : s->ev_free) (void)hipEventDestroy(e);
  if (s->h_pin) (void)hipHostFree(s->h_pin);
  if (s->wave_exec) (void)hipGraphExecDestroy(s->wave_exec);
  if (s->wave_graph) (void)hipGraphDestroy(s->wave_graph);
  if (s->st) (void)hipStreamDestroy(s->st);
  if (s->st2) (void)hipStreamDestroy(s->st2);
  for (int k = 0; k < 4; ++k) {
    if (s->ev_fork[k]) (void)hipEventDestroy(s->ev_fork[k]);
    if (s->ev_join[k]) (void)hipEventDestroy(s->ev_join[k]);
  }
  delete s->xf;
  delete s;
}

static int create_shard(const kb_config* cfg, int rank, int world, Xfer* xf, kb_sim** out) {
  h_crc_init();
  if (!cfg || !out || cfg->abi_version != KB_ABI_VERSION) { seterr("bad config"); delete xf; return KB_INVALID_ARGUMENT; }
  if (cfg->capacity == 0 || cfg->capacity > 7800000u || cfg->initial_nodes > cfg->capacity || cfg->id_len > MAXID ||
      cfg->max_waves == 0 || cfg->max_waves > 64) { seterr("config out of range"); delete xf; return KB_INVALID_ARGUMENT; }
  if (cfg->stat_flags) { seterr("kb_config.stat_flags: sparse rows and the oracle only"); delete xf; return KB_INVALID_ARGUMENT; }
  if (cfg->variant && cfg->variant != KB_VARIANT_EXACT_LRU) { seterr("semantic variants other than KB_VARIANT_SPARSE_ROWS are measurement-only (CPU oracle)"); delete xf; return KB_INVALID_ARGUMENT; }
  const uint32_t C = cfg->capacity;
  const uint32_t rows_per = (C + (uint32_t)world - 1) / (uint32_t)world;
  if (world < 1 || world > (int)XMAX || rank < 0 || rank >= world || (uint64_t)(world - 1) * rows_per >= C) {
    seterr("shard layout out of range (1..8 shards, each holding at least one row)"); delete xf; return KB_INVALID_ARGUMENT;
  }
  int ndev = 0;
  if (hipGetDeviceCount(&ndev) != hipSuccess || ndev == 0) { seterr("no HIP device"); delete xf; return KB_NO_DEVICE; }
  kb_sim* s = new kb_sim();
  memset((void*)&s->d, 0, sizeof s->d);
  memset((void*)&s->xs, 0, sizeof s->xs);
  s->cfg = *cfg;
  s->xf = xf;
  s->rank = rank; s->world = world;
  s->device = cfg->device >= 0 ? cfg->device : 0;
  if (cfg->device < 0) (void)hipGetDevice(&s->device);
  if (hipSetDevice(s->device) != hipSuccess) { destroy_shard(s); seterr("hipSetDevice failed"); return KB_NO_DEVICE; }
  {
    hipDeviceProp_t prop;
    if (hipGetDeviceProperties(&prop, s->device) != hipSuccess) { destroy_shard(s); seterr("hipGetDeviceProperties failed"); return KB_NO_DEVICE; }
    s->ncu = (uint32_t)prop.multiProcessorCount;
    s->lds_per_cu = prop.maxSharedMemoryPerMultiProcessor ? prop.maxSharedMemoryPerMultiProcessor : 65536;
  }
  const uint32_t W = (C + 8191) / 8192 * 8192;
  s->C = C; s->W = W; s->round = 0;
  s->lo = (uint32_t)rank * rows_per;
  s->hi = std::min<uint32_t>(C, s->lo + rows_per);
  s->R = s->hi - s->lo;
  const uint32_t R = s->R;
  const uint32_t groups = (R + 63) / 64;
  uint32_t S = 1;
constexpr uint32_t KB_FOLD_WAVES = 16384;
  while (S < 64 && groups * S < KB_FOLD_WAVES) S <<= 1;
  s->S = S;
  Dev& d = s->d;
  d.lo = s->lo; d.hi = s->hi;
  d.C = C; d.W = W; d.SEGW = W / NSEG; d.NWR = W / 32;
  d.segq = d.SEGW / 128;
  d.segm = d.segq > 1 ? (uint32_t)(((1ull << 32) + d.segq - 1) / d.segq) : 0u;
  d.k0 = (uint32_t)cfg->seed; d.k1 = (uint32_t)(cfg->seed >> 32);
  d.loss_thr = cfg->loss_threshold; d.churn_thr = cfg->churn_threshold; d.fault_end = cfg->fault_end_round;
  d.failed_mode = cfg->failed_mode; d.pgroups = cfg->partition_groups; d.pstart = cfg->partition_start;
  d.pend = cfg->partition_end;
  const uint32_t Lid = cfg->id_len;
  d.capk = (BUFSZ - 20 - Lid) / (18 + Lid);
  d.capj = (BUFSZ - 20 - Lid - 1) / (18 + Lid);
  d.paybound = C < d.capk ? C : d.capk;
  d.dbg = cfg->debug_flags;
  if (const char* dv = getenv("KB_DEV")) d.dev = (uint32_t)atoi(dv);
  s->debug_waves = getenv("KB_DEBUG_WAVES") != nullptr;
  if (const char* gv = getenv("KB_WAVE_GRAPH")) s->graph_on = atoi(gv) != 0;
  if (cfg->debug_flags & KB_DBG_WAVE_GRAPH) s->graph_on = true;
  s->h_ident.assign((size_t)C * MAXID, 0); s->h_idlen.assign(C, (uint8_t)Lid);
  s->h_pend.assign((size_t)C * MAXID, 0); s->h_pendlen.assign(C, (int16_t)-1); s->h_moved.assign(C, 0);
  s->h_idset.assign(C, 0);
  for (uint32_t j = 0; j < C; ++j) default_identity(j, Lid, &s->h_ident[(size_t)j * MAXID]);
  hipError_t e = hipSuccess;
#define A(ptr, n) if (e == hipSuccess) e = talloc(s, &(ptr), (n))
#define AR(ptr, n) if (e == hipSuccess) e = ralloc(s, &(ptr), (n))
  AR(d.stamp, W); AR(d.bits, d.NWR); AR(d.segp, NSEG); AR(d.sdirty, 1);
  AR(d.dirty, 1); A(d.alive, C); A(d.idset, C); A(d.ext, C); A(d.abits, d.NWR); A(d.start_round, C); AR(d.n, 1); AR(d.fp, 1);
  AR(d.last_bcast, 1); AR(d.a3cur, 1); AR(d.susp, SLOTS); AR(d.cur, CSLOTS); AR(d.paq, PAQ);
  AR(d.paq_n, 1); A(d.cseg, C); A(d.segmul, C); A(d.seglen, C); A(d.zpow, (size_t)C + 2); A(d.zfin, (size_t)C + 2);
  A(d.ztab, 17 * 128); A(d.zbtab, ZB);
  A(d.htab, (size_t)(W / 8) * 256); A(d.stats, NSTAT); A(d.sacc, (size_t)NACC * NSTAT); A(d.ctr, NCTR); A(d.truefp, 1); A(d.tfpart, TRUEFP_G);
  AR(d.flog, LOGCAP); AR(d.flog_n, 1); AR(d.fstart, 16); AR(d.kpr_big, 1);
  if (cfg->variant == KB_VARIANT_EXACT_LRU) { AR(d.tst, W); AR(d.tlb, W / 1024); }
  if (cfg->track_latency) { A(d.lat, (size_t)W * lat_stride(R)); A(s->lat_col, C); A(s->fnamed, d.NWR); }
  s->msg_cap = std::max<uint32_t>(8u * R + (uint32_t)TICK_MAX * R, 1u << 16);
  s->pay_cap = std::max<uint32_t>((d.capk + 1) * R, 1u << 24);
  for (int b = 0; b < 2; ++b) {
    A(s->ob[b].msgs, s->msg_cap); A(s->ob[b].pay, s->pay_cap); AR(s->ob[b].off, 1); AR(s->ob[b].cap, 1);
    AR(s->ob[b].cnt, 1); AR(s->ob[b].poff, 1);
    s->ob[b].msg_cap = s->msg_cap; s->ob[b].pay_cap = s->pay_cap;
  }
  AR(s->wc.cnt1, 1); AR(s->wc.bnd, 1); AR(s->wc.bpay, 1); AR(s->wc.cursor, 1);
  AR(s->wc.in_off, 1); A(s->wc.active, R);
  AR(s->wc.kcnt, 1); AR(s->wc.kpay, 1); AR(s->wc.kcur, 1); AR(s->wc.koff, 1);
  if (!xf) { A(s->wc.status, s->msg_cap); A(s->wc.inbox, s->msg_cap); A(s->wc.kin, s->msg_cap); }
  A(s->bfail, (size_t)C * SLOTS); A(s->bjoin, C);
  AR(s->bs.join, 1); AR(s->bs.nfail, 1); AR(s->bs.fail, SLOTS); AR(s->join_off, 1); AR(s->fail_off, 1);
  A(s->scan_tot, 32); A(s->rr, 4); A(s->scan_tiles, 5 * ((std::max<size_t>(C, (size_t)world * R) + 1023) / 1024) + 5);
  AR(s->nresp, 1); AR(s->paysum, 1); AR(s->nbase, 1); AR(s->resp_off, 1);
  A(s->resp_nodes, R); A(s->bf_gid, (size_t)C * SLOTS); A(s->bf_dep, (size_t)C * SLOTS); A(s->slow, R); A(s->defer, R); A(s->w0ctr, W0_WORDS);
  AR(s->ro.part, 10);
  if (xf) {
    XState& x = s->xs;
    x.world = (uint32_t)world; x.R = R; x.S = rows_per; x.RS = R + 1;
    x.NWW = d.NWR; x.nju = 0; x.nj = 0; x.uon = 0;
    s->ucap = std::min<uint32_t>(UCAP, C);
    A(x.ostatus, s->msg_cap); A(x.xcnt, (size_t)world * x.RS); A(x.xpay, (size_t)world * x.RS);
    A(x.xoff, (size_t)world * x.RS); A(x.xpoff, (size_t)world * x.RS); A(x.xb, 2 * world);
    A(x.smsg, (size_t)s->msg_cap + s->ucap); A(x.spay, (size_t)s->pay_cap + (size_t)s->ucap * x.NWW);
    A(x.jslot, C); A(x.ubits, (size_t)s->ucap * x.NWW); A(x.uany, s->ucap);
    A(s->xall, std::max(2 * world * world, 3 * world));
    A(s->xstats, NSTAT);
    A(s->bfail_loc, (size_t)R * SLOTS); A(s->bjoin_loc, R);
    s->h_xall.assign(2 * world * world, 0);
  }
#undef A
#undef AR
  if (e != hipSuccess) { seterr(std::string("device allocation failed: ") + hipGetErrorString(e)); destroy_shard(s); return KB_CAPACITY; }
  (void)hipMemset(L(s, d.kpr_big), 0xFF, 4ull * R);
  if (xf) { (void)hipMemset(s->xs.jslot, 0xFF, 4ull * C); (void)hipMemset(s->xs.ubits, 0, 4ull * s->ucap * s->xs.NWW); }
  if (d.lat) { (void)hipMemset(d.lat, 0xFF, 2ull * lat_stride(R) * W); (void)hipMemset(s->fnamed, 0, 4ull * d.NWR); }
  if (d.tst) {
    (void)hipMemsetD32(d.tst + (size_t)s->lo * W, INT32_MIN / 2, (size_t)R * W);
    (void)hipMemsetD32(d.tlb + (size_t)s->lo * (W / 1024), INT32_MIN, (size_t)R * (W / 1024));
  }
  s->wc.msg_cap = s->msg_cap; s->wc.pay_cap = s->pay_cap;
  if (hipStreamCreateWithFlags(&s->st, hipStreamNonBlocking) != hipSuccess) { destroy_shard(s); seterr("stream"); return KB_IO_ERROR; }
  if (hipStreamCreateWithFlags(&s->st2, hipStreamNonBlocking) != hipSuccess) { destroy_shard(s); seterr("stream"); return KB_IO_ERROR; }
  for (int k = 0; k < 4; ++k)
    if (hipEventCreateWithFlags(&s->ev_fork[k], hipEventDisableTiming) != hipSuccess ||
        hipEventCreateWithFlags(&s->ev_join[k], hipEventDisableTiming) != hipSuccess) { destroy_shard(s); seterr("events"); return KB_IO_ERROR; }
  if (hipHostMalloc((void**)&s->h_pin, 4 * PIN_WORDS, hipHostMallocMapped | hipHostMallocCoherent) != hipSuccess) {
    s->h_pin = nullptr; destroy_shard(s); seterr("pinned buffer"); return KB_IO_ERROR;
  }
  if (hipHostGetDevicePointer((void**)&s->d_pin, s->h_pin, 0) != hipSuccess) { destroy_shard(s); seterr("pinned buffer mapping"); return KB_IO_ERROR; }
  if (const char* pv = getenv("KB_PROF")) s->prof_level = atoi(pv);
  int rc = upload_segments(s);
  if (rc) { destroy_shard(s); return rc; }
  uint32_t ctr0[NCTR] = {0};
  ctr0[C_NEXTFREE] = cfg->initial_nodes;
  ctr0[C_FIRSTCONV] = 0xFFFFFFFFu; ctr0[C_LASTCONV] = 0xFFFFFFFFu;
  if (hipMemcpy(d.ctr, ctr0, sizeof ctr0, hipMemcpyHostToDevice) != hipSuccess) { destroy_shard(s); seterr("ctr upload"); return KB_IO_ERROR; }
  const uint32_t tb = 256, gb = (C + tb - 1) / tb;
  if (cfg->init_mode == KB_INIT_CONVERGED) {
    k_init_converged_rows<<<4096, 256, 0, s->st>>>(d, cfg->initial_nodes);
    k_init_converged_nodes<<<gb, tb, 0, s->st>>>(d, cfg->initial_nodes);
  } else {
    k_init_nodes<<<gb, tb, 0, s->st>>>(d, cfg->initial_nodes);
  }
  if (hipStreamSynchronize(s->st) != hipSuccess) { destroy_shard(s); seterr("init failed"); return KB_IO_ERROR; }
  *out = s;
  return KB_OK;
}

static bool is_group(const kb_sim* s) { return !s->shards.empty(); }
struct Kind { bool sparse, group, rank; };
static Kind kind_of(const kb_sim* s) {
  const kb_sim* f = is_group(s) ? s->shards[0] : s;
  const bool leaf_xf = f->sp ? f->sp->xf != nullptr : f->xf != nullptr;
  return Kind{f->sp != nullptr, is_group(s), !is_group(s) && leaf_xf && !s->in_group};
}
static kb_sim* owner(kb_sim* g, uint32_t node) {
  for (kb_sim* t : g->shards) if (node >= t->lo && node < t->hi) return t;
  return nullptr;
}
template <class F> static int visit(kb_sim* leaf, F&& f) { return leaf->sp ? f(leaf->sp) : f(leaf); }
enum Route { R_ALL, R_OWNER, R_FIRST };
template <class F> static int route(kb_sim* s, Route how, uint32_t node, F&& f) {
  if (!is_group(s)) return visit(s, f);
  if (how != R_ALL) {
    kb_sim* t = how == R_OWNER ? owner(s, node) : s->shards[0];
    (void)hipSetDevice(t->device);
    return visit(t, f);
  }
  for (kb_sim* t : s->shards) {
    (void)hipSetDevice(t->device);
    const int rc = visit(t, f);
    if (rc) return rc;
  }
  return KB_OK;
}

static void destroy_one(kb_sim* s) {
  if (s->sp) { sp_destroy(s->sp); delete s; return; }
  destroy_shard(s);
}

extern "C" int kb_sim_create(const kb_config* cfg, kb_sim** out) {
  if (cfg && out && cfg->abi_version == KB_ABI_VERSION && (cfg->variant & KB_VARIANT_SPARSE_ROWS)) {
    if (cfg->capacity == 0 || cfg->capacity > 7800000u || cfg->initial_nodes > cfg->capacity || cfg->id_len > MAXID ||
        cfg->max_waves == 0 || cfg->max_waves > 64) { seterr("config out of range"); return KB_INVALID_ARGUMENT; }
    return sp_wrap(cfg, 0, 1, nullptr, out);
  }
  return create_shard(cfg, 0, 1, nullptr, out);
}

extern "C" int kb_rccl_unique_id(uint8_t* out, size_t cap) {
  if (!out || cap < sizeof(ncclUniqueId)) { seterr("unique id buffer too small"); return KB_INVALID_ARGUMENT; }
  ncclUniqueId id;
  const ncclResult_t r = ncclGetUniqueId(&id);
  if (r != ncclSuccess) { seterr(std::string("ncclGetUniqueId: ") + ncclGetErrorString(r)); return KB_IO_ERROR; }
  memcpy(out, &id, sizeof id);
  return KB_OK;
}

extern "C" int kb_ipc_unique_id(uint8_t* out, size_t cap) {
  if (!out || cap < KB_UNIQUE_ID_BYTES) { seterr("unique id buffer too small"); return KB_INVALID_ARGUMENT; }
  memset(out, 0, KB_UNIQUE_ID_BYTES);
  memcpy(out, IPC_MAGIC, sizeof IPC_MAGIC);
  uint64_t rnd = 0;
  FILE* f = fopen("/dev/urandom", "rb");
  if (f) { if (fread(&rnd, sizeof rnd, 1, f) != 1) rnd = 0; fclose(f); }
  snprintf(reinterpret_cast<char*>(out) + sizeof IPC_MAGIC, KB_UNIQUE_ID_BYTES - sizeof IPC_MAGIC, "/kbipc-%d-%016llx",
           (int)getpid(), (unsigned long long)rnd);
  return KB_OK;
}

extern "C" int kb_sim_create_rank(const kb_config* cfg, int32_t rank, int32_t world, const uint8_t* unique_id, kb_sim** out) {
  if (!cfg || !unique_id || !out || world < 1 || world > (int)XMAX || rank < 0 || rank >= world) {
    seterr("bad rank/world"); return KB_INVALID_ARGUMENT;
  }
  if (hipSetDevice(cfg->device >= 0 ? cfg->device : 0) != hipSuccess) { seterr("hipSetDevice failed"); return KB_NO_DEVICE; }
  if (memcmp(unique_id, IPC_MAGIC, sizeof IPC_MAGIC) == 0) {
    const char* wm = getenv("KB_IPC_WINDOW_MB");
    const size_t mb = wm ? (size_t)atoll(wm) : 256;
    IpcXfer* x = new IpcXfer();
    if (!x->init(rank, world, unique_id, mb << 20)) { seterr(x->error()); delete x; return KB_IO_ERROR; }
    return (cfg->variant & KB_VARIANT_SPARSE_ROWS) ? sp_wrap(cfg, rank, world, x, out) : create_shard(cfg, rank, world, x, out);
  }
  RcclXfer* x = new RcclXfer();
  if (!x->init(rank, world, unique_id)) { seterr(x->error()); delete x; return KB_IO_ERROR; }
  return (cfg->variant & KB_VARIANT_SPARSE_ROWS) ? sp_wrap(cfg, rank, world, x, out) : create_shard(cfg, rank, world, x, out);
}

extern "C" int kb_sim_create_local(const kb_config* cfg, int32_t shards, kb_sim** out) {
  if (!cfg || !out || shards < 1 || shards > (int)XMAX) { seterr("shards out of range (1..8)"); return KB_INVALID_ARGUMENT; }
  kb_sim* g = new kb_sim();
  g->cfg = *cfg; g->C = cfg->capacity; g->world = shards; g->R = 0;
  g->hub = new LocalHub(shards);
  const bool sparse = cfg->abi_version == KB_ABI_VERSION && (cfg->variant & KB_VARIANT_SPARSE_ROWS);
  for (int k = 0; k < shards; ++k) {
    LocalXfer* x = new LocalXfer();
    x->rank = k; x->world = shards; x->hub = g->hub;
    kb_sim* s = nullptr;
    const int rc = sparse ? sp_wrap(cfg, k, shards, x, &s) : create_shard(cfg, k, shards, x, &s);
    if (rc) { for (kb_sim* t : g->shards) destroy_one(t); delete g->hub; delete g; return rc; }
    s->in_group = true;
    if (s->sp) s->sp->in_group = true;
    g->shards.push_back(s);
  }
  g->device = g->shards[0]->device;
  *out = g;
  return KB_OK;
}

extern "C" int kb_sim_destroy(kb_sim* s) {
  if (!s) return KB_INVALID_ARGUMENT;
  if (!is_group(s)) { destroy_one(s); return KB_OK; }
  for (kb_sim* t : s->shards) destroy_one(t);
  delete s->hub;
  delete s;
  return KB_OK;
}

extern "C" int kb_sim_shard_info(kb_sim* s, int32_t* rank, int32_t* world, uint32_t* lo, uint32_t* hi) {
  if (!s || !rank || !world || !lo || !hi) return KB_INVALID_ARGUMENT;
  if (is_group(s)) { *rank = 0; *world = s->world; *lo = 0; *hi = s->C; return KB_OK; }
  return visit(s, [&](auto* e) { *rank = e->rank; *world = e->world; *lo = e->lo; *hi = e->hi; return KB_OK; });
}

static hipError_t sync_st(kb_sim* s) {
  s->host_syncs++;
  return hipStreamSynchronize(s->st);
}
static int wait_pin(kb_sim* s, uint32_t seq) {
  s->host_syncs++;
  volatile uint32_t* p = s->h_pin + PIN_SEQ;
  for (uint64_t it = 0;; ++it) {
    if (*p == seq) { std::atomic_thread_fence(std::memory_order_acquire); return KB_OK; }
    if ((it & 4095) == 4095) {
      const hipError_t e = hipStreamQuery(s->st);
      if (e == hipSuccess) {
// ... 127 lines not shown
  const std::string e1 = sent ? std::string() : s->xf->error();
  if (!s->xf->group_end() || !sent) { seterr(sent ? s->xf->error() : e1); return KB_IO_ERROR; }
  s->nj = (uint32_t)oj; s->nf = (uint32_t)of;
  return KB_OK;
}

struct RowPlan { bool ldsb, ll; uint32_t wpb; size_t lds; uint32_t per_cu, blocks; };
#include "kb_rounddbg.h"

static int launch_waves(kb_sim* s, int32_t rk) {
  Dev& d = s->d;
  const int32_t r = rk;
  const uint32_t R = s->R;
  hipStream_t st = s->st;
  const uint32_t tb = 256, gnode = (R + tb - 1) / tb;
  int cur = 0;
  for (uint32_t w = 0; w <= s->cfg.max_waves; ++w) {
    OutBuf& ob = s->ob[cur];
    OutBuf& nb = s->ob[cur ^ 1];
    const int last = w == s->cfg.max_waves;
    d.wave = (int32_t)w;
    s->cur_wave = (int)w;
    OutBuf ib = ob;
    uint32_t nrecv = 0;
    if (!s->xf) {
      klaunch(s, KI_ROUTE, k_route, dim3(gnode), dim3(tb), 0, d, ob, s->wc, r, w, last);
      if (last) break;
    } else {
      HIPCHK(hipMemsetAsync(s->xs.xcnt, 0, 4ull * s->world * s->xs.RS, st));
      HIPCHK(hipMemsetAsync(s->xs.xpay, 0, 4ull * s->world * s->xs.RS, st));
      s->xs.nju = w == 0 && !last ? std::min<uint32_t>(s->nj, s->ucap) : 0u;
      s->xs.uon = s->xs.nju && !(d.dbg & KB_DBG_NO_UNION) ? 1u : 0u;
      s->xs.nj = s->xs.uon ? s->nj : 0u;
      s->xs.bjoin = s->bjoin;
      if (s->xs.uon) klaunch(s, KI_ROUTE_X, k_union_slots, dim3((s->xs.nju + 255) / 256), dim3(256), 0, s->xs);
      klaunch(s, KI_ROUTE_X, k_route_x, dim3(gnode), dim3(tb), 0, d, ob, s->xs, r, w, last);
      if (last) break;
      RecvBlocks rb;
      memset(&rb, 0, sizeof rb);
      bool any = true;
      int rc = exchange_wave(s, ob, nrecv, rb, any);
      s->xs.uon = 0;
      if (rc) return rc;
      if (!any) break;
      ib.msgs = s->rmsg; ib.pay = s->rpay;
      if (nrecv) klaunch(s, KI_ROUTE_RECV, k_route_recv, dim3((nrecv + 255) / 256), dim3(256), 0, d, ib, s->wc, rb, nrecv);
    }
    {
      ScanArgs a = scan_args(s, R, s->scan_tot + 8);
      a.narr = 4;
      a.in[0] = L(s, s->wc.cnt1); a.out[0] = L(s, s->wc.in_off);
      a.in[1] = L(s, s->wc.bnd); a.out[1] = L(s, nb.off);
      a.in[2] = L(s, s->wc.bpay); a.out[2] = L(s, nb.poff);
      a.in[3] = L(s, s->wc.kcnt); a.out[3] = L(s, s->wc.koff);
      a.list = s->wc.active; a.list_count = d.ctr + C_ACTIVE; a.list_base = s->lo; a.list_or3 = 1;
      launch_scan(s, a);
    }
    { const int rc = dbg_wave_inboxes(s, r, w); if (rc) return rc; }
    if (!s->xf) klaunch(s, KI_SCATTER, k_scatter, dim3(gnode + PROBE_GROUPS), dim3(tb), 0, d, ob, s->wc, r, gnode);
    else if (nrecv) {
      const uint32_t nsc = (nrecv + 255) / 256;
      klaunch(s, KI_SCATTER_FLAT, k_scatter_flat, dim3(nsc + PROBE_GROUPS), dim3(256), 0, d, ib, s->wc, nrecv, r, nsc);
    }
    { const int rc = dbg_proc_clear(s); if (rc) return rc; }
    const bool split = w == 0 && s->nj > 0 && !s->xf && !s->graph_on && !s->capturing && !s->debug_waves &&
                       !(d.dbg & KB_DBG_WAVE0_SERIAL);
    {
      const uint32_t ks = (d.NWR <= KP_LDS_WORDS && !(d.dbg & KB_DBG_KP_HBM)) ? KP_COLS : 1u;
      const uint32_t groups = std::max<uint32_t>(1u, std::min<uint32_t>((R + 1023) / 1024 * (ks > 1 ? 2u : 1u), 512u / ks));
      constexpr uint32_t KB_KPS_PER_CU = 1;
      const uint32_t small = std::max<uint32_t>((R + 1023) / 1024, KB_KPS_PER_CU * s->ncu);
      if (split) {
        side_fork(s, 3);
        klaunch_on(s, s->st2, KI_KP, k_kp, dim3(ks * groups), dim3(1024), (uint32_t)kp_lds_bytes(d.NWR), d, ib, s->wc, r, nb,
                   ks * groups, (uint32_t*)nullptr);
        side_done(s, 3);
        klaunch(s, KI_KP, k_kp, dim3(small), dim3(1024), 0, d, ib, s->wc, r, nb, 0u, s->w0ctr);
      } else
        klaunch(s, KI_KP, k_kp, dim3(ks * groups + small), dim3(1024), (uint32_t)kp_lds_bytes(d.NWR), d, ib, s->wc, r,
                nb, ks * groups, (uint32_t*)nullptr);
    }
    klaunch(s, KI_SORTFAST, k_sortfast, dim3(SORT_GROUPS + (R + SORTFAST_T - 1) / SORTFAST_T), dim3(SORTFAST_T), 0, d, ib, nb,
            s->wc, r, s->slow, SORT_GROUPS, split ? s->defer : (uint32_t*)nullptr, split ? s->w0ctr : (uint32_t*)nullptr);
    klaunch(s, KI_PROC, k_proc, dim3(std::min<uint32_t>(4096, (KB_PROC_WPE > 2 ? KB_PROC_WPE : 2) * s->ncu)), dim3(256), 0, d, ib, nb, s->wc, r,
            (const uint32_t*)s->slow, (const uint32_t*)(d.ctr + C_SLOW), split ? s->w0ctr + W0_TICKET : (uint32_t*)nullptr);
    if (split) {
      side_join(s, 3);
      klaunch(s, KI_PROC, k_proc, dim3(std::min<uint32_t>(2 * s->ncu, std::max<uint32_t>(1u, (s->nj + 3) / 4))), dim3(256), 0, d, ib, nb,
              s->wc, r, (const uint32_t*)s->defer, (const uint32_t*)(s->w0ctr + W0_DEFER), (uint32_t*)nullptr);
    }
    { const int rc = dbg_proc_report(s, r, w); if (rc) return rc; }
    cur ^= 1;
  }
  s->cur_wave = -1;
  return KB_OK;
}

static int move_row(kb_sim* s, uint32_t from, uint32_t to, bool* snap_after) {
  *snap_after = false;
  const RowPack LP = row_pack_layout(s->W, s->d.NWR, s->d.lat != nullptr, s->d.tst != nullptr);
  if (!s->rpack) { size_t c = 0; const int rc = eng_grow(s, &s->rpack, &c, LP.words); if (rc) return rc; }
  if (s->xf && !s->rpack_in) { size_t c = 0; const int rc = eng_grow(s, &s->rpack_in, &c, LP.words); if (rc) return rc; }
  const bool have = from >= s->lo && from < s->hi, take = to >= s->lo && to < s->hi;
  size_t wk = 0;
  while (wk < s->watch_node.size() && s->watch_node[wk] != from) ++wk;
  const bool watched = have && wk < s->watch_node.size();
  const uint32_t g = (LP.words + 255) / 256 < 1024 ? (LP.words + 255) / 256 : 1024;
  if (have) k_row_pack<<<g, 256, 0, s->st>>>(s->d, from, s->rpack, LP, watched ? s->watch_snap[wk] : nullptr,
                                            watched ? s->watch_fp[wk] : 0u);
  if (watched) { s->watch_node.erase(s->watch_node.begin() + wk); s->watch_fp.erase(s->watch_fp.begin() + wk);
                 s->watch_snap.erase(s->watch_snap.begin() + wk); }
  const uint32_t* src = s->rpack;
  if (s->xf) {
    const int W = s->world, S = (int)s->xs.S;
    const int ofrom = (int)(from / (uint32_t)S), oto = (int)(to / (uint32_t)S);
    size_t sc[XMAX] = {}, sd[XMAX] = {}, rc[XMAX] = {}, rd[XMAX] = {};
    if (s->rank == ofrom) sc[oto] = LP.words;
    if (s->rank == oto) rc[ofrom] = LP.words;
    (void)W;
    if (!s->xf->group_begin()) { seterr(s->xf->error()); return KB_IO_ERROR; }
    const bool sent = s->xf->alltoallv(s->rpack, sc, sd, s->rpack_in, rc, rd, 4, s->st);
    const std::string e1 = sent ? std::string() : s->xf->error();
    if (!s->xf->group_end() || !sent) { seterr(sent ? s->xf->error() : e1); return KB_IO_ERROR; }
    src = s->rpack_in;
  }
  if (!take) return KB_OK;
  uint32_t hdr[RP_HDR];
  HIPCHK(hipMemcpyAsync(hdr, src, sizeof hdr, hipMemcpyDeviceToHost, s->st));
  HIPCHK(sync_st(s));
  uint32_t* snap = nullptr;
  size_t kt = 0;
  while (kt < s->watch_node.size() && s->watch_node[kt] != to) ++kt;
  if (hdr[RP_WATCHED]) {
    if (kt < s->watch_node.size()) { snap = s->watch_snap[kt]; s->watch_fp[kt] = hdr[RP_WFP]; }
    else {
      HIPCHK(talloc(s, &snap, (size_t)s->d.NWR));
      s->watch_node.push_back(to); s->watch_fp.push_back(hdr[RP_WFP]); s->watch_snap.push_back(snap);
    }
  } else if (kt < s->watch_node.size()) {
    *snap_after = true;
  }
  k_row_unpack<<<g, 256, 0, s->st>>>(s->d, to, src, LP, snap);
  return KB_OK;
}

struct Round {
  int32_t r;
  PhaseB pb;
  bool lat_fail = false;
  uint32_t np = 0;
  uint32_t ninj = 0; bool inj_pay = false;
  hipEvent_t er[2] = {nullptr, nullptr};
  size_t krec0 = 0;
};
constexpr uint32_t TB = 256;
static uint32_t gnode(const kb_sim* s) { return (s->R + TB - 1) / TB; }

static int apply_events(kb_sim* s, int32_t r) {
  Dev& d = s->d;
  if (s->events.empty()) return KB_OK;
  { const int rc = round_upload_events(s); if (rc) return rc; }
  size_t k0 = 0;
  for (size_t k = 0; k <= s->events.size(); ++k) {
    const bool rs = k < s->events.size() && s->events[k].kind == EV_RESTART;
    if (k == s->events.size() || rs) {
      if (k > k0) klaunch(s, KI_EVENTS, k_events, dim3(1), dim3(1), 0, d, s->d_events + k0, (uint32_t)(k - k0), r);
      k0 = k;
      if (rs) {
        bool snap_after = false;
        const uint32_t to = s->events[k].node;
        const int rc = move_row(s, s->events[k].src, to, &snap_after);
        if (rc) return rc;
        if (snap_after) {
          klaunch(s, KI_EVENTS, k_events, dim3(1), dim3(1), 0, d, s->d_events + k, 1u, r);
          size_t kt = 0;
          while (s->watch_node[kt] != to) ++kt;
          k_events_commit<<<(d.NWR + 255) / 256, 256, 0, s->st>>>(d.bits + (size_t)to * d.NWR, s->watch_snap[kt], d.NWR);
          k0 = k + 1;
        }
      }
    }
  }
  HIPCHK(sync_st(s));
  s->events.clear();
  return KB_OK;
}
static int round_lifecycle(kb_sim* s, Round& q) {
  Dev& d = s->d;
  const int32_t r = q.r;
  if (r > 0 && r % EPOCH == 0) klaunch(s, KI_REBASE, k_rebase, dim3(8192), dim3(256), 0, d, r);
  { const int rc = apply_events(s, r); if (rc) return rc; }
  const bool faults_on = s->cfg.fault_end_round < 0 || r < s->cfg.fault_end_round;
  if (faults_on && s->cfg.churn_threshold) {
    klaunch(s, KI_CHURN_LEAVE, k_churn_leave, dim3((s->C + TB - 1) / TB), dim3(TB), 0, d, r);
    klaunch(s, KI_CHURN_JOIN, k_churn_join, dim3(1), dim3(64), 0, d, r);
  }
  klaunch(s, KI_LOG_MARK, k_log_mark, dim3(gnode(s)), dim3(TB), 0, d, r);
  return KB_OK;
}

template <class F> static void rowpass_with(const RowPlan& p, F&& f) {
  if (p.ldsb) { if (p.ll) f(k_rowpass<true, true>); else f(k_rowpass<true, false>); }
  else if (p.ll) f(k_rowpass<false, true>);
  else f(k_rowpass<false, false>);
}
static RowPlan rowpass_plan(kb_sim* s, bool pb_hbm) {
  const Dev& d = s->d;
  RowPlan p;
  const uint32_t budget = RP_LDS_BYTES / 4;
  p.ll = s->nf <= PB_FMAX && s->nj <= PB_JMAX;
  uint32_t listw = p.ll ? 2 * s->nf + s->nj : 0;
  if (listw > budget / 2 || pb_hbm) { p.ll = false; listw = 0; }
  p.ldsb = s->W <= PB_LDS_W && budget - listw >= d.NWR && !pb_hbm && s->nf > 0;
  p.wpb = p.ldsb ? std::min<uint32_t>(RP_WAVES, (budget - listw) / d.NWR) : RP_WAVES;
  p.lds = 4ull * ((p.ldsb ? (size_t)p.wpb * d.NWR : 0) + listw);
  int occ = 0;
  const uint64_t okey = ((uint64_t)p.ldsb << 63) | ((uint64_t)p.ll << 62) | ((uint64_t)p.wpb << 40) | (uint64_t)p.lds;
  if (okey == s->occ_key) occ = s->occ_val;
  else {
    rowpass_with(p, [&](auto k) { (void)hipOccupancyMaxActiveBlocksPerMultiprocessor(&occ, reinterpret_cast<const void*>(k), (int)(64 * p.wpb), p.lds); });
    s->occ_key = okey; s->occ_val = occ;
  }
  p.per_cu = std::max<uint32_t>(1, std::min<uint32_t>(8, (uint32_t)occ));
  p.blocks = std::min<uint32_t>((s->R + p.wpb - 1) / p.wpb, s->ncu * p.per_cu);
  return p;
}

static int round_broadcasts(kb_sim* s, Round& q) {
  Dev& d = s->d;
  const int32_t r = q.r;
  const uint32_t R = s->R;
  if (!s->inj_join.empty()) { const int rc = merge_ext_joins(s->st, s->bjoin, &s->nj, s->inj_join, 0, s->C); if (rc) return rc; }
  PhaseB& pb = q.pb;
  pb.bfail = s->bfail; pb.nf = s->nf; pb.bjoin = s->bjoin; pb.nj = s->nj; pb.JW = (s->nj + 63) / 64;
  pb.nresp = s->nresp; pb.paysum = s->paysum; pb.nbase = s->nbase;
  if (pb.JW) {
    const size_t words = (size_t)R * pb.JW;
    if (words > s->mask_words) {
      const int rc = eng_grow_group(s, &s->mask_words, words, words, &s->newmask_base, &s->respmask_base);
      if (rc) return rc;
    }
    s->newmask = bias(s->newmask_base, pb.JW, s->lo);
    s->respmask = bias(s->respmask_base, pb.JW, s->lo);
  }
  pb.newmask = s->newmask; pb.respmask = s->respmask;
  pb.gid = s->bf_gid; pb.dep = s->bf_dep;
  q.lat_fail = d.lat && s->nf && d.failed_mode == KB_FAILED_SIM_SENDER;
  pb.fnamed = q.lat_fail ? s->fnamed : nullptr;
  if (q.lat_fail) klaunch(s, KI_LAT_MARK, k_lat_mark, dim3((s->nf + 255) / 256), dim3(256), 0, (const BCast*)s->bfail, s->nf, s->fnamed);
  const bool pb_hbm = (d.dbg & KB_DBG_PHASEB_HBM) != 0;
  if (s->nf > BFAIL_LDS_MAX || (pb_hbm && s->nf)) klaunch(s, KI_BFAIL_PREP, k_bfail_prep, dim3((s->nf + 255) / 256), dim3(256), 0, (const BCast*)s->bfail, s->nf, s->bf_gid, s->bf_dep, d.ctr + C_PATHS);
  else if (s->nf) klaunch(s, KI_BFAIL_PREP, k_bfail_prep_lds, dim3(1), dim3(1024), 0, (const BCast*)s->bfail, s->nf, s->bf_gid, s->bf_dep);
  { const int rc = dbg_bcast_shape(s, r); if (rc) return rc; }
  {
    const RowPlan p = rowpass_plan(s, pb_hbm);
    { const int rc = dbg_rowpass_begin(s, r, p); if (rc) return rc; }
    if (p.ldsb && !p.ll) s->host_paths |= PATH_ROWPASS_LDS_HBM_LISTS;
    rowpass_with(p, [&](auto k) { klaunch(s, KI_ROWPASS, k, dim3(p.blocks), dim3(64 * p.wpb), (uint32_t)p.lds, d, pb, s->ro, r); });
    { const int rc = dbg_rowpass_shares(s, r, p); if (rc) return rc; }
  }
  side_fork(s, 0);
  klaunch_on(s, s->st2, KI_ALIVE_BITS, k_alive_bits, dim3((d.NWR + TB - 1) / TB), dim3(TB), 0, d);
  klaunch_on(s, s->st2, KI_TRUEFP_PART, k_truefp_part, dim3(TRUEFP_G), dim3(256), 0, d, d.tfpart);
  klaunch_on(s, s->st2, KI_TRUEFP_FIN, k_truefp_fin, dim3(1), dim3(64), 0, d, d.tfpart);
  side_done(s, 0);
  if (q.lat_fail) {
    klaunch_on(s, s->st2, KI_LAT_SWEEP, k_lat_sweep, dim3((lat_stride(R) / 8 + 255) / 256, std::min<uint32_t>(s->nf, 16384)), dim3(256), 0, d,
            (const BCast*)s->bfail, (const uint32_t*)s->bf_gid, s->nf, s->fnamed);
    side_done(s, 1);
  }
  { const int rc = round_take_probes(s, R, &q.np); if (rc) return rc; }
  if (q.np) klaunch(s, KI_PROBE, k_probe, dim3(gnode(s)), dim3(TB), 0, d, q.np, r, s->d_presp, s->d_presp_n, (uint32_t)s->presp_cap);
  return KB_OK;
}

static int launch_join_responses(kb_sim* s, Round& q, uint32_t resp_nodes) {
  Dev& d = s->d;
  const int32_t r = q.r;
  OutBuf& o0 = s->ob[0];
  const uint32_t grid = std::min<uint32_t>(resp_nodes, 4096);
  const size_t words = resp_words(d.NWR, s->W / 256);
  uint32_t* scratch = nullptr;
  size_t lds = 4 * words;
  const bool resp_hbm = s->W > RESP_LDS_W || (d.dbg & KB_DBG_RESP_HBM);
  if (resp_hbm) {
    { const int rc = eng_grow(s, &s->resp_scratch, &s->resp_scratch_words, words * grid); if (rc) return rc; }
    scratch = s->resp_scratch;
    lds = 0;
  }
  const size_t wlds = 16ull * rwave_words(d.NWR, s->W / 256);
  const size_t hlds = 4ull * rwave_head(s->W / 256);
  const bool full_on = wlds <= 65536 && !(d.dbg & (KB_DBG_RESP_HBM | KB_DBG_RESP_WAVE_HBM));
  const uint32_t hwaves = (uint32_t)std::min<size_t>(4, 65536 / hlds);
  const bool head_on = !full_on && hwaves >= 1 && !(d.dbg & KB_DBG_RESP_HBM);
  const bool wave_on = full_on || head_on;
  { const int rc = dbg_resp_clear(s); if (rc) return rc; }
  if (full_on) {
    klaunch(s, KI_RESP_WAVE, k_resp_wave<false>, dim3(std::min<uint32_t>((resp_nodes + 3) / 4, 4096)), dim3(256), (uint32_t)wlds, d,
            q.pb, (const uint32_t*)s->resp_nodes, (const uint32_t*)(s->scan_tot + 4), o0, r, s->slow);
  } else if (head_on) {
    klaunch(s, KI_RESP_WAVE, k_resp_wave<true>, dim3(std::min<uint32_t>((resp_nodes + hwaves - 1) / hwaves, 4096)),
            dim3(64 * hwaves), (uint32_t)(hwaves * hlds), d, q.pb, (const uint32_t*)s->resp_nodes,
            (const uint32_t*)(s->scan_tot + 4), o0, r, s->slow);
  }
  klaunch(s, KI_RESP_NODE, k_resp_node, dim3(wave_on ? std::min<uint32_t>(grid, 2 * s->ncu) : grid), dim3(256), (uint32_t)lds, d, q.pb,
          (const uint32_t*)(wave_on ? s->slow : s->resp_nodes), (const uint32_t*)(wave_on ? d.ctr + C_RESTN : s->scan_tot + 4),
          o0, r, scratch, wave_on);
  return dbg_resp_report(s, r);
}

static int round_wave0_regions(kb_sim* s, Round& q) {
  Dev& d = s->d;
  const int32_t r = q.r;
  const uint32_t R = s->R;
  OutBuf& o0 = s->ob[0];
  q.ninj = (uint32_t)s->inj.size();
  if (q.ninj) {
    if (q.ninj > s->d_inj_cap) { const int rc = eng_grow(s, &s->d_inj, &s->d_inj_cap, 2 * (size_t)q.ninj); if (rc) return rc; }
    if (s->inj_ids.size() > s->d_inj_ids_cap || !s->d_inj_ids) {
      const int rc = eng_grow(s, &s->d_inj_ids, &s->d_inj_ids_cap, 2 * s->inj_ids.size() + 16);
      if (rc) return rc;
    }
    HIPCHK(hipMemcpyAsync(s->d_inj, s->inj.data(), sizeof(XRec) * q.ninj, hipMemcpyHostToDevice, s->st));
    if (!s->inj_ids.empty()) {
      HIPCHK(hipMemcpyAsync(s->d_inj_ids, s->inj_ids.data(), 4 * s->inj_ids.size(), hipMemcpyHostToDevice, s->st));
      q.inj_pay = true;
    }
    klaunch(s, KI_EVENTS, k_inject_prep, dim3(1), dim3(64), 0, d, (const XRec*)s->d_inj, q.ninj, s->paysum);
  }
  {
    ScanArgs a = scan_args(s, R, s->scan_tot);
    a.narr = 3;
    a.in[0] = L(s, s->nresp); a.out[0] = L(s, s->resp_off);
    a.in[1] = L(s, s->paysum); a.out[1] = L(s, o0.poff);
    a.in[2] = L(s, s->nresp); a.out[2] = L(s, o0.off); a.addc[2] = TICK_MAX;
    a.list = s->resp_nodes; a.list_base = s->lo;
    launch_scan(s, a);
  }
  const bool need_tot = s->nj > 0 || q.inj_pay;
  klaunch(s, KI_SET_CAP, k_set_cap, dim3(gnode(s)), dim3(TB), 0, d, s->nresp, o0.cap, o0.cnt, s->scan_tot, s->d_pin, need_tot ? ++s->pin_seq : 0u);
  if (!need_tot) return KB_OK;
  const uint32_t* tot = s->h_pin;
  { const int rc = wait_pin(s, s->pin_seq); if (rc) return rc; }
  const uint32_t pay_tot = tot[1], msg_tot = tot[2], resp_nodes = tot[4];
  if (msg_tot > o0.msg_cap || pay_tot > o0.pay_cap) { const int rc = grow_wave0(s, msg_tot, pay_tot); if (rc) return rc; }
  if (s->n_ext) { const int rc = round_size_exports(s, msg_tot, pay_tot); if (rc) return rc; }
  return resp_nodes ? launch_join_responses(s, q, resp_nodes) : KB_OK;
}

static int round_tick(kb_sim* s, Round& q) {
  Dev& d = s->d;
  const int32_t r = q.r;
  const uint32_t R = s->R, gn = gnode(s);
  OutBuf& o0 = s->ob[0];
  if (q.lat_fail) side_join(s, 1);
  klaunch(s, KI_TICK_SCAN, k_tick_scan, dim3(gn), dim3(TB), 0, d, s->bs, r, s->slow);
  klaunch(s, KI_TICK_PRE, k_tick_pre, dim3(std::min<uint32_t>((R + 3) / 4, 1024)), dim3(256), 0, d, o0, s->bs, r, s->slow);
  if (d.tst) {
    side_fork(s, 2);
    const uint32_t kpl = a3_kpl(s->W, d.dbg);
    if (kpl == 2) klaunch_on(s, s->st2, KI_A3_EXACT, k_a3_exact<2>, dim3((R + 3) / 4), dim3(256), 0, d, s->ro.part, r);
    else if (kpl) klaunch_on(s, s->st2, KI_A3_EXACT, k_a3_exact<A3X_KPL>, dim3((R + 3) / 4), dim3(256), 0, d, s->ro.part, r);
    else klaunch_on(s, s->st2, KI_A3_EXACT, k_a3_exact<0>, dim3((R + 3) / 4), dim3(256), 0, d, s->ro.part, r);
    side_done(s, 2);
  }
  if (d.uniform) klaunch(s, KI_FOLD, k_fold, dim3(((R + 63) / 64 + 3) / 4 * s->S), dim3(256), 0, d, FoldArgs{s->S});
  if (d.uniform) klaunch(s, KI_FP_ROWS, k_fp_rows, dim3((FP_LANES * R + TB - 1) / TB), dim3(TB), 0, d);
  side_join(s, 0);
  if (d.tst) side_join(s, 2);
  klaunch(s, KI_TICK_POST, k_tick_post, dim3(gn), dim3(TB), 0, d, s->ro, o0, r);
  if (q.ninj) {
    klaunch(s, KI_EVENTS, k_inject, dim3(1), dim3(64), 0, d, o0, (const XRec*)s->d_inj, q.ninj, (const uint32_t*)s->d_inj_ids);
    s->inj.clear(); s->inj_ids.clear();
  }
  {
    ScanArgs a = scan_args(s, R, s->scan_tot);
    a.narr = 2;
    a.in[0] = L(s, s->bs.join); a.out[0] = L(s, s->join_off);
    a.in[1] = L(s, s->bs.nfail); a.out[1] = L(s, s->fail_off);
    launch_scan(s, a);
  }
  klaunch(s, KI_BCAST_WRITE, k_bcast_write, dim3(gn), dim3(TB), 0, d, s->bs, (const uint32_t*)s->join_off,
          (const uint32_t*)s->fail_off, s->xf ? s->bjoin_loc : s->bjoin, s->xf ? s->bfail_loc : s->bfail);
  return KB_OK;
}

static int round_window(kb_sim* s, Round& q) {
  hipStream_t st = s->st;
  if (s->xf || s->debug_waves || !s->graph_on) return launch_waves(s, q.r);
  if (!s->wave_exec || s->wave_gen != s->buf_gen) {
    if (s->wave_exec) { (void)hipGraphExecDestroy(s->wave_exec); s->wave_exec = nullptr; }
    if (s->wave_graph) { (void)hipGraphDestroy(s->wave_graph); s->wave_graph = nullptr; }
    HIPCHK(hipStreamBeginCapture(st, hipStreamCaptureModeThreadLocal));
    s->capturing = true;
    const int rc = launch_waves(s, -1);
    s->capturing = false;
    hipGraph_t g = nullptr;
    const hipError_t e = hipStreamEndCapture(st, &g);
    if (rc) { if (g) (void)hipGraphDestroy(g); return rc; }
    HIPCHK(e);
    s->wave_graph = g;
    HIPCHK(hipGraphInstantiate(&s->wave_exec, g, nullptr, nullptr, 0));
    s->wave_gen = s->buf_gen;
  }
  HIPCHK(hipGraphLaunch(s->wave_exec, st));
  return KB_OK;
}

static int round_finish(kb_sim* s, Round& q) {
  Dev& d = s->d;
  const int32_t r = q.r;
  hipStream_t st = s->st;
  if (s->xf && !s->xf->allreduce_sum_u32(d.ctr + C_AGREE, 1, st)) { seterr(s->xf->error()); return KB_IO_ERROR; }
  klaunch(s, KI_ROUND_END, k_round_end, dim3(1), dim3(1), 0, d, r, (const uint32_t*)s->scan_tot, s->d_pin,
          s->xf ? 0u : ++s->pin_seq, s->rr);
  (void)hipEventRecord(q.er[1], st);
  s->krec.push_back(kb_sim::KRec{(int16_t)NKI, (int16_t)-1, q.er[0], q.er[1]});
  prof_resolve(s, q.krec0);
  uint32_t err = 0;
  if (s->xf) {
    const int rc = gather_broadcasts(s, &err);
    if (rc) return rc;
  } else {
    const int rc = wait_pin(s, s->pin_seq);
    if (rc) return rc;
    s->nj = s->h_pin[0]; s->nf = s->h_pin[1]; err = s->h_pin[2];
  }
  s->bj_total += s->nj; s->bf_total += s->nf;
  { const int rc = round_drain_exports(s); if (rc) return rc; }
  { const int rc = round_drain_probes(s, q.np, r); if (rc) return rc; }
  s->round = r + 1;
  return err_status(err);
}

static int step_round(kb_sim* s) {
  Round q;
  q.r = s->round;
  q.krec0 = s->krec.size();
  s->cur_wave = -1;
  for (int k = 0; k < 2; ++k) {
    if (!s->ev_free.empty()) { q.er[k] = s->ev_free.back(); s->ev_free.pop_back(); }
    else (void)hipEventCreate(&q.er[k]);
  }
  (void)hipEventRecord(q.er[0], s->st);
  int rc = round_lifecycle(s, q);
  if (!rc) rc = round_broadcasts(s, q);
  if (!rc) rc = round_wave0_regions(s, q);
  if (!rc) rc = round_tick(s, q);
  if (!rc) rc = round_window(s, q);
  if (!rc) rc = round_finish(s, q);
  return rc;
}

static int group_step(kb_sim* g, uint32_t rounds) {
  const size_t W = g->shards.size();
  std::vector<int> rc(W, KB_OK);
  std::vector<std::string> err(W);
  g->hub->reset();
  std::vector<std::thread> th;
  for (size_t k = 0; k < W; ++k)
    th.emplace_back([&, k] {
      kb_sim* s = g->shards[k];
      (void)hipSetDevice(s->device);
      for (uint32_t q = 0; q < rounds && rc[k] == KB_OK; ++q) rc[k] = s->sp ? sp_step(s->sp, 1) : step_round(s);
      if (rc[k] == KB_OK && !s->sp && sync_st(s) != hipSuccess) { rc[k] = KB_IO_ERROR; g_err = "stream"; }
      if (rc[k] != KB_OK) { err[k] = g_err; g->hub->abort(); }
    });
  for (auto& t : th) t.join();
  int first = KB_OK;
  for (int pass = 0; pass < 2 && first == KB_OK; ++pass)
    for (size_t k = 0; k < W && first == KB_OK; ++k)
      if (rc[k] != KB_OK && (pass == 1 || err[k].find("aborted by another shard") == std::string::npos)) {
        first = rc[k];
        seterr(err[k]);
      }
  return first;
}

extern "C" int kb_sim_step(kb_sim* s, uint32_t rounds) {
  if (!s) return KB_INVALID_ARGUMENT;
  if (s->probed) { seterr("the handle ran the fold probe (kb_sim_debug_fold): it cannot step"); return KB_INVALID_OPERATION; }
  if (is_group(s)) return group_step(s, rounds);
  if (s->sp) return sp_step(s->sp, rounds);
  (void)hipSetDevice(s->device);
  for (uint32_t k = 0; k < rounds; ++k) {
    int rc = step_round(s);
    if (rc) { if (s->xf) s->xf->abort(); return rc; }
  }
  HIPCHK(sync_st(s));
  return KB_OK;
}

static int chk(kb_sim* s, uint32_t node) { return (!s || node >= s->C) ? KB_INVALID_ARGUMENT : KB_OK; }
static int read_row(kb_sim* s, uint32_t node, std::vector<uint8_t>& rw) {
  std::vector<uint32_t> bw(s->d.NWR);
  rw.resize(s->C);
  HIPCHK(hipMemcpy(rw.data(), s->d.stamp + (size_t)node * s->W, s->C, hipMemcpyDeviceToHost));
  HIPCHK(hipMemcpy(bw.data(), s->d.bits + (size_t)node * s->d.NWR, 4ull * s->d.NWR, hipMemcpyDeviceToHost));
  for (uint32_t j = 0; j < s->C; ++j) if (!((bw[j >> 5] >> (j & 31)) & 1u)) rw[j] = 0;
  return KB_OK;
}

#include "kb_ctl.h"

static int mark_all_dirty(kb_sim* s) {
  k_mark_all_dirty<<<(s->R + 255) / 256, 256, 0, s->st>>>(s->d);
  HIPCHK(hipStreamSynchronize(s->st));
  return KB_OK;
}
static void window_stale(kb_sim* s) { s->buf_gen++; }
static int export_alloc(kb_sim* s) {
  s->d.xrec_cap = XREC_MIN; s->d.xids_cap = XIDS_MIN;
  HIPCHK(talloc(s, &s->d.xrec, s->d.xrec_cap)); HIPCHK(talloc(s, &s->d.xids, s->d.xids_cap));
  window_stale(s);
  return KB_OK;
}
static int row_fp(kb_sim* s, uint32_t node, uint32_t* fp) {
  if (ctl_chk_row(s, node)) return KB_INVALID_ARGUMENT;
  k_fp_one<<<1, 64, 0, s->st>>>(s->d, node);
  HIPCHK(hipMemcpyAsync(fp, s->d.fp + node, 4, hipMemcpyDeviceToHost, s->st));
  HIPCHK(hipStreamSynchronize(s->st));
  return KB_OK;
// ... 541 lines not shown
```

kaboodle_amd/csrc/kb_tick.h:

```cpp
#pragma once
#include "kb_common.h"

namespace kb {

struct BcastSlots { uint32_t* join; uint32_t* nfail; uint32_t* fail; };

__device__ __attribute__((always_inline)) inline void tick_a2(const Dev& d, const OutBuf& ob, const BcastSlots& bs, int32_t r,
                                                              uint32_t i, uint32_t l, uint32_t* pr, uint32_t* pp,
                                                              uint32_t* pid) {
  uint32_t n = d.n[i];
  Susp* sl = d.susp + (size_t)i * SLOTS;
  const Susp me = l < SLOTS ? sl[l] : Susp{0, 0, 0, 0};
  const bool occ = l < SLOTS && me.kind != 0;
  const unsigned long long occm = __ballot(occ);
  const unsigned long long tim = __ballot(occ && r - me.since >= PING_TIMEOUT);
  if (!tim) { if (l == 0) bs.nfail[i] = 0; return; }
  const uint32_t nsusp = __popcll(occm);
  const uint32_t m = n - 1 - nsusp;
  uint32_t myrank = 0;
  for (int k = 0; k < SLOTS; ++k) if (((occm >> k) & 1ull) && rdl(me.peer, k) < me.peer) myrank++;
  uint32_t npick = 0, nind = 0, nrem = 0;
  uint32_t indirect[SLOTS], removed[SLOTS];
  for (uint32_t t = 0; t < nsusp; ++t) {
    const unsigned long long who = __ballot(occ && myrank == t);
    const int k = __ffsll((long long)who) - 1;
    const uint32_t peer = rdl(me.peer, k);
    const int32_t kind = (int32_t)rdl((uint32_t)me.kind, k), since = (int32_t)rdl((uint32_t)me.since, k);
    if (r - since < PING_TIMEOUT) continue;
    if (kind == SK_WFP) {
      const uint32_t kk = m < (uint32_t)NUM_INDIRECT ? m : (uint32_t)NUM_INDIRECT;
      if (kk == 0) { removed[nrem++] = peer; continue; }
      const U4 w = philox(i, (uint32_t)r, (uint32_t)P_INDIRECT << 24, peer, d.k0, d.k1);
      uint32_t pk[3];
      pk[0] = mulhi(w.x, m);
      if (kk > 1) { const uint32_t b = mulhi(w.y, m - 1); pk[1] = b + (b >= pk[0]); }
      if (kk > 2) {
        const uint32_t lo = pk[0] < pk[1] ? pk[0] : pk[1], hi = pk[0] < pk[1] ? pk[1] : pk[0];
        uint32_t c = mulhi(w.z, m - 2);
        if (c >= lo) c++;
        if (c >= hi) c++;
        pk[2] = c;
      }
      if (l == 0) for (uint32_t q = 0; q < kk; ++q) { pr[npick + q] = pk[q]; pp[npick + q] = peer; pid[npick + q] = 0xFFFFFFFFu; }
      npick += kk;
      indirect[nind++] = peer;
    } else {
      removed[nrem++] = peer;
    }
  }
  uint32_t oseq = ob.cnt[i];
  if (npick) {
    wait_lds();
    __builtin_amdgcn_wave_barrier();
    const uint4* b4 = reinterpret_cast<const uint4*>(bits_of(d, i));
    uint32_t ex[SLOTS + 1];
    ex[0] = i;
#pragma unroll
    for (int k = 0; k < SLOTS; ++k) ex[k + 1] = ((occm >> k) & 1ull) ? rdl(me.peer, k) : 0xFFFFFFFFu;
    uint32_t maxrank = 0;
    for (uint32_t q = 0; q < npick; ++q) maxrank = pr[q] > maxrank ? pr[q] : maxrank;
    const uint32_t n4 = d.NWR / 4;
    uint32_t base = 0;
    constexpr int PB = 8;
    for (uint32_t w0 = 0; w0 < n4 && base <= maxrank; w0 += 64 * PB) {
      uint4 v[PB];
#pragma unroll
      for (int u = 0; u < PB; ++u) { const uint32_t w = w0 + 64u * u + l; v[u] = w < n4 ? b4[w] : make_uint4(0, 0, 0, 0); }
#pragma unroll
      for (int u = 0; u < PB; ++u) {
        if (base > maxrank) break;
        const uint32_t w = w0 + 64u * u + l, id0 = w * 128;
        const uint32_t wd[4] = {v[u].x, v[u].y, v[u].z, v[u].w};
        uint32_t c = __popc(wd[0]) + __popc(wd[1]) + __popc(wd[2]) + __popc(wd[3]);
#pragma unroll
        for (int k = 0; k <= SLOTS; ++k) c -= (ex[k] - id0 < 128u) ? 1u : 0u;
        const uint32_t exl = wave_excl(c), tot = wave_sum(c);
        for (uint32_t q = 0; q < npick; ++q) {
          const uint32_t rk = pr[q];
          if (rk >= base + exl && rk < base + exl + c) {
            uint32_t rem = rk - base - exl, id = 0xFFFFFFFFu;
#pragma unroll
            for (int k = 0; k < 4; ++k) {
              uint32_t m = wd[k];
#pragma unroll
              for (int e = 0; e <= SLOTS; ++e) if ((ex[e] >> 5) == w * 4 + k) m &= ~(1u << (ex[e] & 31));
              const uint32_t pc = __popc(m);
              if (id == 0xFFFFFFFFu) { if (rem < pc) id = id0 + 32 * k + select_in_word(m, rem); else rem -= pc; }
            }
            pid[q] = id;
          }
        }
        base += tot;
      }
    }
    wait_lds();
    __builtin_amdgcn_wave_barrier();
    for (uint32_t q = 0; q < npick; ++q) emit_msg(ob, d, i, oseq, pid[q], K_PINGREQ, pp[q], 0, 0, 0);
  }
  if (l == 0) {
    for (uint32_t q = 0; q < nind; ++q)
      for (int k = 0; k < SLOTS; ++k) if (sl[k].kind && sl[k].peer == indirect[q]) { sl[k].kind = SK_WFIP; sl[k].since = r; }
    Cur* cu = d.cur + (size_t)i * CSLOTS;
    unsigned long long segs = 0;
    for (uint32_t q = 0; q < nrem; ++q) {
      const uint32_t p = removed[q];
      susp_clear(d, i, p);
      mem_clr(d, i, p);
      lat_none(d, i, p);
      segs |= seg_bit(d, p);
      n--;
      for (int c = 0; c < CSLOTS; ++c) if (cu[c].used && cu[c].peer == p) cu[c].used = 0;
      bs.fail[(size_t)i * SLOTS + q] = p;
    }
    bs.nfail[i] = nrem;
    if (nrem) { d.n[i] = n; mark(d, i, segs); slot_add(d, S_RMTIMEOUT, nrem); }
    ob.cnt[i] = oseq;
  }
}

__global__ __launch_bounds__(256) void k_tick_scan(Dev d, BcastSlots bs, int32_t r, uint32_t* list) {
  const uint32_t i = d.lo + blockIdx.x * blockDim.x + threadIdx.x;
  if (i >= d.hi) return;
  if (!d.alive[i]) { bs.join[i] = 0; bs.nfail[i] = 0; return; }
  const int32_t lb = d.last_bcast[i];
  uint32_t j = 0;
  if (lb == NONE_ROUND || (r - lb >= REBROADCAST && d.n[i] <= 1)) { j = 1; d.last_bcast[i] = r; }
  bs.join[i] = j;
  const Susp* sl = d.susp + (size_t)i * SLOTS;
  bool tim = false;
#pragma unroll
  for (int k = 0; k < SLOTS; ++k) { const Susp x = sl[k]; tim |= x.kind != 0 && r - x.since >= PING_TIMEOUT; }
  if (!tim) { bs.nfail[i] = 0; return; }
  const unsigned long long m = __ballot(true);
  const int first = __ffsll((long long)m) - 1;
  uint32_t base = 0;
  if (lane() == (uint32_t)first) base = atomicAdd(&d.ctr[C_TICK], (uint32_t)__popcll(m));
  list[rdl(base, first) + __popcll(m & ((1ull << lane()) - 1ull))] = i;
}

__global__ __launch_bounds__(256) void k_tick_pre(Dev d, OutBuf ob, BcastSlots bs, int32_t r, const uint32_t* list) {
  __shared__ uint32_t s_pick_rank[4][SLOTS * 3], s_pick_peer[4][SLOTS * 3], s_pick_id[4][SLOTS * 3];
  const uint32_t wv = threadIdx.x >> 6;
  const uint32_t l = lane();
  const uint32_t nlist = d.ctr[C_TICK];
  for (uint32_t it = blockIdx.x * 4 + wv; it < nlist; it += gridDim.x * 4) {
    tick_a2(d, ob, bs, r, list[it], l, s_pick_rank[wv], s_pick_peer[wv], s_pick_id[wv]);
  }
}


struct FoldArgs { uint32_t S; };

__global__ __launch_bounds__(256) void k_fold(Dev d, FoldArgs fa) {
  __shared__ uint32_t zb[ZB];
  load_zbtab(d, zb);
  const uint32_t S = fa.S;
  const uint32_t s = blockIdx.x % S;
  const uint32_t g = (blockIdx.x / S) * 4 + (threadIdx.x >> 6);
  const uint32_t i0 = d.lo + g * 64 + lane();
  const bool act = i0 < d.hi && d.alive[i0] && d.uniform;
  const unsigned long long actm = __ballot(act);
  __shared__ uint32_t s_nb[4];
  uint32_t nbytes = 0;
  if (actm) {
    const uint32_t i = act ? i0 : d.lo + g * 64 + (uint32_t)(__ffsll((long long)actm) - 1);
    const uint32_t* bw = bits_of(d, i);
    const uint32_t spp = NSEG / S;
    const unsigned long long sd = act ? d.sdirty[i] : 0ull;
    unsigned long long folded = 0;
    for (uint32_t k = s * spp; k < (s + 1) * spp; ++k) {
      const bool mine = (sd >> k) & 1ull;
      if (!__ballot(mine)) continue;
      const uint32_t c0 = k * d.SEGW, c1 = c0 + d.SEGW;
      uint32_t raw = 0, cnt = 0;
      uint4 mb = *reinterpret_cast<const uint4*>(bw + (c0 >> 5));
      for (uint32_t col = c0; col < c1; col += 128) {
        const uint32_t mw[4] = {mb.x, mb.y, mb.z, mb.w};
        uint32_t hv[16];
        const uint32_t* ht = d.htab + (size_t)(col >> 3) * 256;
#pragma unroll
        for (int h = 0; h < 16; ++h) hv[h] = ht[h * 256 + ((mw[h >> 2] >> (8 * (h & 3))) & 0xFFu)];
        if (col + 128 < c1) mb = *reinterpret_cast<const uint4*>(bw + ((col + 128) >> 5));
#pragma unroll
        for (int h = 0; h < 16; ++h) {
          const uint32_t c = __popc((mw[h >> 2] >> (8 * (h & 3))) & 0xFFu);
          raw = mulzb(zb, raw, c) ^ hv[h];
          cnt += c;
        }
      }
      if (mine) { d.segp[(size_t)i * NSEG + k] = make_uint2(raw, cnt); folded |= 1ull << k; nbytes += d.SEGW / 8; }
    }
    if (folded) atomicAnd(&d.sdirty[i], ~folded);
  }
  const uint32_t wb = wave_sum(act ? nbytes : 0u);
  if (lane() == 0) s_nb[threadIdx.x >> 6] = wb;
  __syncthreads();
  if (threadIdx.x == 0) {
    const uint32_t t = s_nb[0] + s_nb[1] + s_nb[2] + s_nb[3];
    if (t) slot_add(d, S_FOLDB, t);
  }
}

constexpr uint32_t KB_FP_LANES = 8;
constexpr uint32_t FP_LANES = KB_FP_LANES;
__global__ __launch_bounds__(256) void k_fp_rows(Dev d) {
  constexpr uint32_t PER = NSEG / FP_LANES;
  const uint32_t t = blockIdx.x * blockDim.x + threadIdx.x;
  const uint32_t i = d.lo + t / FP_LANES, part = t % FP_LANES;
  const bool on = i < d.hi && d.uniform && d.alive[i] && d.dirty[i];
  uint32_t raw = 0, cnt = 0;
  if (on) {
    const uint4* sp4 = reinterpret_cast<const uint4*>(d.segp + (size_t)i * NSEG + PER * part);
    uint4 q[PER / 2];
#pragma unroll
    for (uint32_t k = 0; k < PER / 2; ++k) q[k] = sp4[k];
    uint32_t z[PER];
#pragma unroll
    for (uint32_t k = 0; k < PER; ++k) { const uint32_t c = (k & 1) ? q[k >> 1].w : q[k >> 1].y; z[k] = c ? d.zpow[c] : 0u; }
#pragma unroll
    for (uint32_t k = 0; k < PER; ++k) {
      const uint32_t x = (k & 1) ? q[k >> 1].z : q[k >> 1].x, c = (k & 1) ? q[k >> 1].w : q[k >> 1].y;
      if (c) { raw = multmodp(z[k], raw) ^ x; cnt += c; }
    }
  }
  static_assert(FP_LANES == 8, "the combine below is three DPP levels inside a 16-lane row");
  auto level = [&](uint32_t r2, uint32_t c2, uint32_t st) __attribute__((always_inline)) {
    if (on && (part & (2 * st - 1)) == 0) { raw = multmodp(d.zpow[c2], raw) ^ r2; cnt += c2; }
  };
  { const uint32_t r2 = dpp_shl<1>(raw), c2 = dpp_shl<1>(cnt); level(r2, c2, 1); }
  { const uint32_t r2 = dpp_shl<2>(raw), c2 = dpp_shl<2>(cnt); level(r2, c2, 2); }
  { const uint32_t r2 = dpp_shl<4>(raw), c2 = dpp_shl<4>(cnt); level(r2, c2, 4); }
  if (on && part == 0) { d.fp[i] = finish_fp(d, raw, cnt); d.dirty[i] = 0; }
}

__global__ void k_tick_post(Dev d, RowOut ro, OutBuf ob, int32_t r) {
  const uint32_t i = d.lo + blockIdx.x * blockDim.x + threadIdx.x;
  unsigned long long agree = 0;
  if (i < d.hi && d.alive[i]) {
    const uint32_t C = d.C;
    const uint32_t cur = d.a3cur[i];
    const uint32_t p = (cur + 1 == C) ? 0 : cur + 1;
    uint32_t k5[5];
    const uint4 a = *reinterpret_cast<const uint4*>(ro.part + (size_t)i * 10);
    k5[0] = a.x; k5[1] = a.y; k5[2] = a.z; k5[3] = a.w; k5[4] = ro.part[(size_t)i * 10 + 4];
    uint32_t nc = 0;
    while (nc < 5 && k5[nc] != 0xFFFFFFFFu) nc++;
    uint32_t oseq = ob.cnt[i];
    if (nc) {
      const uint32_t u = philox(i, (uint32_t)r, (uint32_t)P_PING << 24, 0, d.k0, d.k1).x;
      const uint32_t rot = k5[mulhi(u, nc)] & 0xFFFFFFu;
      const uint32_t t = rot + p >= C ? rot + p - C : rot + p;
      const uint32_t rot0 = k5[0] & 0xFFFFFFu;
      const uint32_t c1 = rot0 + p >= C ? rot0 + p - C : rot0 + p;
      d.a3cur[i] = c1 == 0 ? C - 1 : c1 - 1;
      Susp* sl = d.susp + (size_t)i * SLOTS;
      int k = 0;
      while (k < SLOTS && sl[k].kind) ++k;
      if (k == SLOTS) set_err(d, DERR_SLOTS);
      else { sl[k].peer = t; sl[k].kind = SK_WFP; sl[k].since = r; }
      uint8_t* tb = row_of(d, i) + t;
      if (*tb == enc(r, r)) {
        const uint32_t e = log_entry(t, r), fe = d.flog_n[i];
        for (uint32_t q = d.fstart[(size_t)i * 16 + ((uint32_t)r & 15u)]; q < fe; ++q) {
          uint32_t& slot = d.flog[(size_t)i * LOGCAP + (q & (LOGCAP - 1))];
          if (slot == e) slot = LOG_INVALID;
        }
      }
      *tb = ST_SUSPECT;
      if (oseq >= ob.cap[i]) set_err(d, DERR_OUTBOX);
      else ob.msgs[ob.off[i] + oseq] = Msg{t, i, oseq, K_PING, 0, 0, 0, 0};
      oseq++;
    }
    const uint32_t pn = d.paq_n[i];
    for (uint32_t q = 0; q < pn; ++q) {
      const uint32_t t = d.paq[(size_t)i * PAQ + q];
      if (oseq >= ob.cap[i]) set_err(d, DERR_OUTBOX);
      else ob.msgs[ob.off[i] + oseq] = Msg{t, i, oseq, K_PING, 0, 0, 0, 0};
      oseq++;
    }
    d.paq_n[i] = 0;
    ob.cnt[i] = oseq;
    thread_refresh_fp(d, i);
    agree = d.fp[i] == d.truefp[0];
  }
  const unsigned long long t = block_sum(agree);
  if (threadIdx.x == 0 && t) atomicAdd(&d.ctr[C_AGREE], (uint32_t)t);
}

__global__ void k_bcast_write(Dev d, BcastSlots bs, const uint32_t* join_off, const uint32_t* fail_off, BCast* bjoin,
                              BCast* bfail) {
  const uint32_t i = d.lo + blockIdx.x * blockDim.x + threadIdx.x;
  if (i >= d.hi) return;
  uint32_t bseq = 0;
  if (bs.join[i]) bjoin[join_off[i]] = BCast{i, i, bseq++, 0};
  const uint32_t nfl = bs.nfail[i];
  for (uint32_t q = 0; q < nfl; ++q) bfail[fail_off[i] + q] = BCast{i, bs.fail[(size_t)i * SLOTS + q], bseq++, 0};
}

__global__ void k_inject_prep(Dev d, const XRec* inj, uint32_t n, uint32_t* paysum) {
// ... 36 lines not shown
```

Baseline: 12.74 million.

## Split join responses by tick-timeout flag and overlap independent half on side stream

Runs the tick scan before the join-response kernels and marks nodes with pending suspect timeouts. Responses for unflagged nodes go on a third stream while flagged nodes are handled on the main stream ahead of the tick pre-pass, which lets the response work overlap tick processing. The response kernels now batch node indices per wave via ballot to filter by phase. This adds extra launches, a second rest list and a stream/event pair. It also risks ordering hazards, since the side-stream responses run alongside tick work that mutates node rows.

```diff
diff --git a/include/kaboodle_sim.h b/include/kaboodle_sim.h
--- a/include/kaboodle_sim.h
+++ b/include/kaboodle_sim.h
@@ -65,7 +65,8 @@
   KB_DBG_NO_UNION = 128u,
   KB_DBG_A3X_KPL8 = 256u,
   KB_DBG_A3X_WIDE = 512u,
-  KB_DBG_WAVE0_SERIAL = 1024u
+  KB_DBG_WAVE0_SERIAL = 1024u,
+  KB_DBG_RESP_SERIAL = 2048u
 };
 
 enum { KB_STATE_KNOWN = 0, KB_STATE_WAITING_FOR_PING = 1, KB_STATE_WAITING_FOR_INDIRECT_PING = 2 };
diff --git a/kaboodle_amd/_ffi.py b/kaboodle_amd/_ffi.py
--- a/kaboodle_amd/_ffi.py
+++ b/kaboodle_amd/_ffi.py
@@ -16,6 +16,7 @@
 KB_DBG_A3X_KPL8 = 256
 KB_DBG_A3X_WIDE = 512
 KB_DBG_WAVE0_SERIAL = 1024
+KB_DBG_RESP_SERIAL = 2048
 KB_VARIANT_SAME_WINDOW_BCAST, KB_VARIANT_EXACT_LRU = 1, 2
 KB_STAT_NO_SF_FAILED_DROPS = 1
 KB_VARIANT_SPARSE_ROWS = 4
diff --git a/kaboodle_amd/csrc/kb_common.h b/kaboodle_amd/csrc/kb_common.h
--- a/kaboodle_amd/csrc/kb_common.h
+++ b/kaboodle_amd/csrc/kb_common.h
@@ -40,7 +40,9 @@
                   PATH_ROWPASS_LDS_HBM_LISTS = 1024,
                   PATH_KPR_WRAPPED = 2048,
                   PATH_RESP_JOINERS_HBM = 4096,
-                  PATH_JOIN_LIST_PAST_UCAP = 8192 };
+                  PATH_JOIN_LIST_PAST_UCAP = 8192,
+                  PATH_RESP_PHASE1 = 16384,
+                  PATH_A2_RESPONDER = 32768 };
 constexpr int NSEG = 64;
 constexpr int ZT = 9;
 constexpr int ZB = 9 * 1024;
diff --git a/kaboodle_amd/csrc/kb_round.h b/kaboodle_amd/csrc/kb_round.h
--- a/kaboodle_amd/csrc/kb_round.h
+++ b/kaboodle_amd/csrc/kb_round.h
@@ -1128,9 +1128,13 @@
 __device__ inline bool resp_by_wave(const Dev& d, uint32_t i, uint32_t nnew, bool on) {
   return on && d.uniform && nnew <= RW_JCAP && d.n[i] - nnew > d.capj;
 }
+__device__ inline bool resp_phase_serves(uint32_t phase, const uint8_t* a2flag, uint32_t i) {
+  return phase == 0 || (a2flag[i] != 0) == (phase == 1);
+}
 template <bool SG>
 __global__ __launch_bounds__(256) __attribute__((amdgpu_waves_per_eu(4))) void k_resp_wave(Dev d, PhaseB pb, const uint32_t* nodes, const uint32_t* nnodes_p,
-                                                   OutBuf ob, int32_t r, uint32_t* rest) {
+                                                   OutBuf ob, int32_t r, uint32_t* rest, uint32_t* restn, uint32_t phase,
+                                                   const uint8_t* a2flag) {
   extern __shared__ __attribute__((aligned(16))) uint32_t rw_lds[];
   const uint32_t NW = d.NWR, NB = d.W / 256;
   const uint32_t wv = threadIdx.x >> 6, l = lane(), nwv = blockDim.x >> 6;
@@ -1142,16 +1146,19 @@
   const uint32_t js0 = small_lists && l < pb.nj ? pb.bjoin[l].sender : 0u;
   const uint32_t js1 = small_lists && l + 64 < pb.nj ? pb.bjoin[l + 64].sender : 0u;
   const uint32_t stride = gridDim.x * nwv;
-  uint32_t it = blockIdx.x * nwv + wv;
-  uint32_t inext = it < nnodes ? nodes[it] : 0u;
-  for (; it < nnodes; it += stride) {
-    const uint32_t i = inext;
+  for (uint32_t it0 = blockIdx.x * nwv + wv; it0 < nnodes; it0 += 64 * stride) {
+   const uint32_t itl = it0 + l * stride;
+   const uint32_t node_l = itl < nnodes ? nodes[itl] : 0u;
+   unsigned long long todo = __ballot(itl < nnodes && resp_phase_serves(phase, a2flag, node_l));
+   while (todo) {
+    const int tb = __ffsll((long long)todo) - 1;
+    todo &= todo - 1;
+    const uint32_t i = rdl(node_l, tb);
     const unsigned long long* nm = pb.newmask + (size_t)i * pb.JW;
     const unsigned long long* rm = pb.respmask + (size_t)i * pb.JW;
     const unsigned long long nmv = small_lists && l < pb.JW ? nm[l] : 0ull;
     const unsigned long long rmv = small_lists && l < pb.JW ? rm[l] : 0ull;
     const uint32_t n_i = d.n[i], nbase_i = pb.nbase[i], poff_i = ob.poff[i], ooff_i = ob.off[i];
-    inext = it + stride < nnodes ? nodes[it + stride] : 0u;
     const uint32_t* B = bits_of(d, i);
     const uint4* B4 = reinterpret_cast<const uint4*>(B);
     const bool tdbg = (d.dev & 512) != 0;
@@ -1161,12 +1168,13 @@
     if (small_lists) nnew = wave_sum((uint32_t)__popcll(nmv));
     else for (uint32_t wj = 0; wj < pb.JW; ++wj) nnew += __popcll(nm[wj]);
     if (!(d.uniform && nnew <= RW_JCAP && n_i - nnew > d.capj)) {
-      if (l == 0) rest[atomicAdd(&d.ctr[C_RESTN], 1u)] = i;
+      if (l == 0) rest[atomicAdd(restn, 1u)] = i;
       wait_lds();
       __builtin_amdgcn_wave_barrier();
       continue;
     }
     if (l == 0) path_hit(d, SG ? PATH_RESP_WAVE_HBM : PATH_RESP_WAVE);
+    if (l == 0 && phase == 1) path_hit(d, PATH_RESP_PHASE1);
     uint64_t tp0 = tdbg ? wall_clock64() : 0, tp1 = 0, tp2 = 0;
     if (small_lists) {
       const unsigned long long w0 = ((unsigned long long)rdl((uint32_t)(nmv >> 32), 0) << 32) | rdl((uint32_t)nmv, 0);
@@ -1257,11 +1265,13 @@
     }
     wait_lds();
     __builtin_amdgcn_wave_barrier();
+   }
   }
 }
 
 __global__ __launch_bounds__(256) void k_resp_node(Dev d, PhaseB pb, const uint32_t* nodes, const uint32_t* nnodes_p,
-                                                   OutBuf ob, int32_t r, uint32_t* gscratch, bool wave_on) {
+                                                   OutBuf ob, int32_t r, uint32_t* gscratch, bool wave_on, uint32_t phase,
+                                                   const uint8_t* a2flag) {
   extern __shared__ uint32_t lds_dyn[];
   const uint32_t NW = d.NWR, NB = d.W / 256;
   uint32_t* lds = gscratch ? gscratch + (size_t)blockIdx.x * resp_words(NW, NB) : lds_dyn;
@@ -1276,6 +1286,7 @@
   const uint32_t nnodes = *nnodes_p;
   for (uint32_t it = blockIdx.x; it < nnodes; it += gridDim.x) {
     const uint32_t i = nodes[it];
+    if (!resp_phase_serves(phase, a2flag, i)) continue;
     const unsigned long long* nm = pb.newmask + (size_t)i * pb.JW;
     const unsigned long long* rm = pb.respmask + (size_t)i * pb.JW;
     uint32_t nnew = 0;
@@ -1367,6 +1378,7 @@
           ob.msgs[ob.off[i] + q] = m;
           if (nk != expect) set_err(d, DERR_RESP);
           if (gscratch) path_hit(d, sample ? PATH_RESP_SCRATCH_SAMPLED : PATH_RESP_SCRATCH_FULL);
+          if (phase == 1) path_hit(d, PATH_RESP_PHASE1);
           if (!jl) path_hit(d, PATH_RESP_JOINERS_HBM);
         }
         poff += cap; q++;
diff --git a/kaboodle_amd/csrc/kb_sim.hip b/kaboodle_amd/csrc/kb_sim.hip
--- a/kaboodle_amd/csrc/kb_sim.hip
+++ b/kaboodle_amd/csrc/kb_sim.hip
@@ -121,10 +121,10 @@
   d.htab[k] = raw;
 }
 __global__ void k_set_cap(Dev d, const uint32_t* nresp, uint32_t* cap, uint32_t* cnt, const uint32_t* tot, uint32_t* hpin,
-                          uint32_t seq) {
+                          uint32_t seq, uint32_t* rest2n) {
   const uint32_t i = d.lo + blockIdx.x * blockDim.x + threadIdx.x;
   if (i < d.hi) { cap[i] = nresp[i] + TICK_MAX; cnt[i] = nresp[i]; }
-  if (blockIdx.x == 0 && threadIdx.x == 0) { d.ctr[C_RESTN] = 0; pin_publish(hpin, tot, 5, seq); }
+  if (blockIdx.x == 0 && threadIdx.x == 0) { d.ctr[C_RESTN] = 0; *rest2n = 0; pin_publish(hpin, tot, 5, seq); }
 }
 __global__ void k_publish(const uint32_t* v, uint32_t n, uint32_t* hpin, uint32_t seq) {
   if (blockIdx.x == 0 && threadIdx.x == 0) pin_publish(hpin, v, n, seq);
@@ -297,7 +297,8 @@
   int device;
   hipStream_t st;
   hipStream_t st2 = nullptr;
-  hipEvent_t ev_fork[4] = {nullptr, nullptr, nullptr, nullptr}, ev_join[4] = {nullptr, nullptr, nullptr, nullptr};
+  hipStream_t st3 = nullptr;
+  hipEvent_t ev_fork[5] = {nullptr, nullptr, nullptr, nullptr, nullptr}, ev_join[5] = {nullptr, nullptr, nullptr, nullptr, nullptr};
   uint32_t C, W, S;
   uint32_t lo, hi, R;
   int rank, world;
@@ -338,6 +339,9 @@
   uint32_t* nresp; uint32_t* paysum; uint32_t* nbase; uint32_t* resp_off;
   uint32_t* resp_nodes; uint32_t* bf_gid; uint8_t* bf_dep;
   uint32_t* slow;
+  uint32_t* rest[2] = {nullptr, nullptr};
+  uint32_t* rest2n = nullptr;
+  uint8_t* a2flag = nullptr;
   uint32_t* defer = nullptr;
   uint32_t* w0ctr = nullptr;
   uint16_t* lat_col;
@@ -433,8 +437,9 @@
 static void klaunch(kb_sim* s, int kid, F kern, dim3 grid, dim3 block, uint32_t lds, Args... args) {
   klaunch_on(s, s->st, kid, kern, grid, block, lds, args...);
 }
-static void side_fork(kb_sim* s, int k) { (void)hipEventRecord(s->ev_fork[k], s->st); (void)hipStreamWaitEvent(s->st2, s->ev_fork[k], 0); }
-static void side_done(kb_sim* s, int k) { (void)hipEventRecord(s->ev_join[k], s->st2); }
+static hipStream_t side_stream(kb_sim* s, int k) { return k == 4 ? s->st3 : s->st2; }
+static void side_fork(kb_sim* s, int k) { (void)hipEventRecord(s->ev_fork[k], s->st); (void)hipStreamWaitEvent(side_stream(s, k), s->ev_fork[k], 0); }
+static void side_done(kb_sim* s, int k) { (void)hipEventRecord(s->ev_join[k], side_stream(s, k)); }
 static void side_join(kb_sim* s, int k) { (void)hipStreamWaitEvent(s->st, s->ev_join[k], 0); }
 static void prof_resolve(kb_sim* s, size_t n) {
   n = std::min(n, s->krec.size());
@@ -561,7 +566,8 @@
   if (s->wave_graph) (void)hipGraphDestroy(s->wave_graph);
   if (s->st) (void)hipStreamDestroy(s->st);
   if (s->st2) (void)hipStreamDestroy(s->st2);
-  for (int k = 0; k < 4; ++k) {
+  if (s->st3) (void)hipStreamDestroy(s->st3);
+  for (int k = 0; k < 5; ++k) {
     if (s->ev_fork[k]) (void)hipEventDestroy(s->ev_fork[k]);
     if (s->ev_join[k]) (void)hipEventDestroy(s->ev_join[k]);
   }
@@ -659,6 +665,7 @@
   A(s->scan_tot, 32); A(s->rr, 4); A(s->scan_tiles, 5 * ((std::max<size_t>(C, (size_t)world * R) + 1023) / 1024) + 5);
   AR(s->nresp, 1); AR(s->paysum, 1); AR(s->nbase, 1); AR(s->resp_off, 1);
   A(s->resp_nodes, R); A(s->bf_gid, (size_t)C * SLOTS); A(s->bf_dep, (size_t)C * SLOTS); A(s->slow, R); A(s->defer, R); A(s->w0ctr, W0_WORDS);
+  A(s->rest[0], R); A(s->rest[1], R); A(s->rest2n, 1); AR(s->a2flag, 1);
   AR(s->ro.part, 10);
   if (xf) {
     XState& x = s->xs;
@@ -687,7 +694,8 @@
   s->wc.msg_cap = s->msg_cap; s->wc.pay_cap = s->pay_cap;
   if (hipStreamCreateWithFlags(&s->st, hipStreamNonBlocking) != hipSuccess) { destroy_shard(s); seterr("stream"); return KB_IO_ERROR; }
   if (hipStreamCreateWithFlags(&s->st2, hipStreamNonBlocking) != hipSuccess) { destroy_shard(s); seterr("stream"); return KB_IO_ERROR; }
-  for (int k = 0; k < 4; ++k)
+  if (hipStreamCreateWithFlags(&s->st3, hipStreamNonBlocking) != hipSuccess) { destroy_shard(s); seterr("stream"); return KB_IO_ERROR; }
+  for (int k = 0; k < 5; ++k)
     if (hipEventCreateWithFlags(&s->ev_fork[k], hipEventDisableTiming) != hipSuccess ||
         hipEventCreateWithFlags(&s->ev_join[k], hipEventDisableTiming) != hipSuccess) { destroy_shard(s); seterr("events"); return KB_IO_ERROR; }
   if (hipHostMalloc((void**)&s->h_pin, 4 * PIN_WORDS, hipHostMallocMapped | hipHostMallocCoherent) != hipSuccess) {
@@ -1121,6 +1129,8 @@
   uint32_t ninj = 0; bool inj_pay = false;
   hipEvent_t er[2] = {nullptr, nullptr};
   size_t krec0 = 0;
+  bool tick_scanned = false;
+  bool resp_side = false;
 };
 constexpr uint32_t TB = 256;
 static uint32_t gnode(const kb_sim* s) { return (s->R + TB - 1) / TB; }
@@ -1243,15 +1253,20 @@
   return KB_OK;
 }
 
-static int launch_join_responses(kb_sim* s, Round& q, uint32_t resp_nodes) {
+static bool resp_rows_hbm(const kb_sim* s) { return s->W > RESP_LDS_W || (s->d.dbg & KB_DBG_RESP_HBM); }
+static int launch_join_responses(kb_sim* s, Round& q, uint32_t resp_nodes, uint32_t phase) {
   Dev& d = s->d;
   const int32_t r = q.r;
   OutBuf& o0 = s->ob[0];
+  hipStream_t st = phase == 2 ? s->st3 : s->st;
+  uint32_t* rest = s->rest[phase == 2];
+  uint32_t* restn = phase == 2 ? s->rest2n : d.ctr + C_RESTN;
+  const uint32_t wcap = phase == 1 ? s->ncu : 4096;
   const uint32_t grid = std::min<uint32_t>(resp_nodes, 4096);
   const size_t words = resp_words(d.NWR, s->W / 256);
   uint32_t* scratch = nullptr;
   size_t lds = 4 * words;
-  const bool resp_hbm = s->W > RESP_LDS_W || (d.dbg & KB_DBG_RESP_HBM);
+  const bool resp_hbm = resp_rows_hbm(s);
   if (resp_hbm) {
     { const int rc = eng_grow(s, &s->resp_scratch, &s->resp_scratch_words, words * grid); if (rc) return rc; }
     scratch = s->resp_scratch;
@@ -1265,17 +1280,24 @@
   const bool wave_on = full_on || head_on;
   { const int rc = dbg_resp_clear(s); if (rc) return rc; }
   if (full_on) {
-    klaunch(s, KI_RESP_WAVE, k_resp_wave<false>, dim3(std::min<uint32_t>((resp_nodes + 3) / 4, 4096)), dim3(256), (uint32_t)wlds, d,
-            q.pb, (const uint32_t*)s->resp_nodes, (const uint32_t*)(s->scan_tot + 4), o0, r, s->slow);
+    klaunch_on(s, st, KI_RESP_WAVE, k_resp_wave<false>, dim3(std::min<uint32_t>((resp_nodes + 3) / 4, wcap)), dim3(256), (uint32_t)wlds, d,
+               q.pb, (const uint32_t*)s->resp_nodes, (const uint32_t*)(s->scan_tot + 4), o0, r, rest, restn, phase, (const uint8_t*)s->a2flag);
   } else if (head_on) {
-    klaunch(s, KI_RESP_WAVE, k_resp_wave<true>, dim3(std::min<uint32_t>((resp_nodes + hwaves - 1) / hwaves, 4096)),
-            dim3(64 * hwaves), (uint32_t)(hwaves * hlds), d, q.pb, (const uint32_t*)s->resp_nodes,
-            (const uint32_t*)(s->scan_tot + 4), o0, r, s->slow);
-  }
-  klaunch(s, KI_RESP_NODE, k_resp_node, dim3(wave_on ? std::min<uint32_t>(grid, 2 * s->ncu) : grid), dim3(256), (uint32_t)lds, d, q.pb,
-          (const uint32_t*)(wave_on ? s->slow : s->resp_nodes), (const uint32_t*)(wave_on ? d.ctr + C_RESTN : s->scan_tot + 4),
-          o0, r, scratch, wave_on);
+    klaunch_on(s, st, KI_RESP_WAVE, k_resp_wave<true>, dim3(std::min<uint32_t>((resp_nodes + hwaves - 1) / hwaves, wcap)),
+               dim3(64 * hwaves), (uint32_t)(hwaves * hlds), d, q.pb, (const uint32_t*)s->resp_nodes,
+               (const uint32_t*)(s->scan_tot + 4), o0, r, rest, restn, phase, (const uint8_t*)s->a2flag);
+  }
+  klaunch_on(s, st, KI_RESP_NODE, k_resp_node, dim3(wave_on ? std::min<uint32_t>(grid, 2 * s->ncu) : grid), dim3(256), (uint32_t)lds, d, q.pb,
+             (const uint32_t*)(wave_on ? rest : s->resp_nodes), (const uint32_t*)(wave_on ? restn : s->scan_tot + 4),
+             o0, r, scratch, wave_on, phase, (const uint8_t*)s->a2flag);
   return dbg_resp_report(s, r);
+}
+static bool resp_overlap_on(const kb_sim* s) {
+  return !s->xf && !resp_rows_hbm(s) && !s->debug_waves && !(s->d.dbg & KB_DBG_RESP_SERIAL);
+}
+static void launch_tick_scan(kb_sim* s, Round& q) {
+  klaunch(s, KI_TICK_SCAN, k_tick_scan, dim3(gnode(s)), dim3(TB), 0, s->d, s->bs, q.r, s->slow, s->a2flag);
+  q.tick_scanned = true;
 }
 
 static int round_wave0_regions(kb_sim* s, Round& q) {
@@ -1307,14 +1329,22 @@
     launch_scan(s, a);
   }
   const bool need_tot = s->nj > 0 || q.inj_pay;
-  klaunch(s, KI_SET_CAP, k_set_cap, dim3(gnode(s)), dim3(TB), 0, d, s->nresp, o0.cap, o0.cnt, s->scan_tot, s->d_pin, need_tot ? ++s->pin_seq : 0u);
+  klaunch(s, KI_SET_CAP, k_set_cap, dim3(gnode(s)), dim3(TB), 0, d, s->nresp, o0.cap, o0.cnt, s->scan_tot, s->d_pin, need_tot ? ++s->pin_seq : 0u,
+          s->rest2n);
   if (!need_tot) return KB_OK;
   const uint32_t* tot = s->h_pin;
   { const int rc = wait_pin(s, s->pin_seq); if (rc) return rc; }
   const uint32_t pay_tot = tot[1], msg_tot = tot[2], resp_nodes = tot[4];
   if (msg_tot > o0.msg_cap || pay_tot > o0.pay_cap) { const int rc = grow_wave0(s, msg_tot, pay_tot); if (rc) return rc; }
   if (s->n_ext) { const int rc = round_size_exports(s, msg_tot, pay_tot); if (rc) return rc; }
-  return resp_nodes ? launch_join_responses(s, q, resp_nodes) : KB_OK;
+  if (!resp_nodes) return KB_OK;
+  if (!resp_overlap_on(s)) return launch_join_responses(s, q, resp_nodes, 0);
+  launch_tick_scan(s, q);
+  side_fork(s, 4);
+  { const int rc = launch_join_responses(s, q, resp_nodes, 2); if (rc) return rc; }
+  side_done(s, 4);
+  q.resp_side = true;
+  return launch_join_responses(s, q, resp_nodes, 1);
 }
 
 static int round_tick(kb_sim* s, Round& q) {
@@ -1323,8 +1353,9 @@
   const uint32_t R = s->R, gn = gnode(s);
   OutBuf& o0 = s->ob[0];
   if (q.lat_fail) side_join(s, 1);
-  klaunch(s, KI_TICK_SCAN, k_tick_scan, dim3(gn), dim3(TB), 0, d, s->bs, r, s->slow);
-  klaunch(s, KI_TICK_PRE, k_tick_pre, dim3(std::min<uint32_t>((R + 3) / 4, 1024)), dim3(256), 0, d, o0, s->bs, r, s->slow);
+  if (!q.tick_scanned) launch_tick_scan(s, q);
+  klaunch(s, KI_TICK_PRE, k_tick_pre, dim3(std::min<uint32_t>((R + 3) / 4, 1024)), dim3(256), 0, d, o0, s->bs, r, s->slow,
+          (const uint32_t*)s->nresp);
   if (d.tst) {
     side_fork(s, 2);
     const uint32_t kpl = a3_kpl(s->W, d.dbg);
@@ -1337,6 +1368,7 @@
   if (d.uniform) klaunch(s, KI_FP_ROWS, k_fp_rows, dim3((FP_LANES * R + TB - 1) / TB), dim3(TB), 0, d);
   side_join(s, 0);
   if (d.tst) side_join(s, 2);
+  if (q.resp_side) side_join(s, 4);
   klaunch(s, KI_TICK_POST, k_tick_post, dim3(gn), dim3(TB), 0, d, s->ro, o0, r);
   if (q.ninj) {
     klaunch(s, KI_EVENTS, k_inject, dim3(1), dim3(64), 0, d, o0, (const XRec*)s->d_inj, q.ninj, (const uint32_t*)s->d_inj_ids);
diff --git a/kaboodle_amd/csrc/kb_tick.h b/kaboodle_amd/csrc/kb_tick.h
--- a/kaboodle_amd/csrc/kb_tick.h
+++ b/kaboodle_amd/csrc/kb_tick.h
@@ -7,7 +7,7 @@
 
 __device__ __attribute__((always_inline)) inline void tick_a2(const Dev& d, const OutBuf& ob, const BcastSlots& bs, int32_t r,
                                                               uint32_t i, uint32_t l, uint32_t* pr, uint32_t* pp,
-                                                              uint32_t* pid) {
+                                                              uint32_t* pid, const uint32_t* nresp) {
   uint32_t n = d.n[i];
   Susp* sl = d.susp + (size_t)i * SLOTS;
   const Susp me = l < SLOTS ? sl[l] : Susp{0, 0, 0, 0};
@@ -114,13 +114,15 @@
     }
     bs.nfail[i] = nrem;
     if (nrem) { d.n[i] = n; mark(d, i, segs); slot_add(d, S_RMTIMEOUT, nrem); }
+    if (nrem && nresp[i]) path_hit(d, PATH_A2_RESPONDER);
     ob.cnt[i] = oseq;
   }
 }
 
-__global__ __launch_bounds__(256) void k_tick_scan(Dev d, BcastSlots bs, int32_t r, uint32_t* list) {
+__global__ __launch_bounds__(256) void k_tick_scan(Dev d, BcastSlots bs, int32_t r, uint32_t* list, uint8_t* a2flag) {
   const uint32_t i = d.lo + blockIdx.x * blockDim.x + threadIdx.x;
   if (i >= d.hi) return;
+  a2flag[i] = 0;
   if (!d.alive[i]) { bs.join[i] = 0; bs.nfail[i] = 0; return; }
   const int32_t lb = d.last_bcast[i];
   uint32_t j = 0;
@@ -136,15 +138,17 @@
   uint32_t base = 0;
   if (lane() == (uint32_t)first) base = atomicAdd(&d.ctr[C_TICK], (uint32_t)__popcll(m));
   list[rdl(base, first) + __popcll(m & ((1ull << lane()) - 1ull))] = i;
-}
-
-__global__ __launch_bounds__(256) void k_tick_pre(Dev d, OutBuf ob, BcastSlots bs, int32_t r, const uint32_t* list) {
+  a2flag[i] = 1;
+}
+
+__global__ __launch_bounds__(256) void k_tick_pre(Dev d, OutBuf ob, BcastSlots bs, int32_t r, const uint32_t* list,
+                                                  const uint32_t* nresp) {
   __shared__ uint32_t s_pick_rank[4][SLOTS * 3], s_pick_peer[4][SLOTS * 3], s_pick_id[4][SLOTS * 3];
   const uint32_t wv = threadIdx.x >> 6;
   const uint32_t l = lane();
   const uint32_t nlist = d.ctr[C_TICK];
   for (uint32_t it = blockIdx.x * 4 + wv; it < nlist; it += gridDim.x * 4) {
-    tick_a2(d, ob, bs, r, list[it], l, s_pick_rank[wv], s_pick_peer[wv], s_pick_id[wv]);
+    tick_a2(d, ob, bs, r, list[it], l, s_pick_rank[wv], s_pick_peer[wv], s_pick_id[wv], nresp);
   }
 }
 
```

After: 13.10 million, median of 6. 1.03x the previous value.
